# ai-forever/Kandinsky-2

Measured on AMD Instinct MI355X. Metric: UNet denoise steps/sec @ 768x768 bs=1, 50 steps, higher is better.
Workload: dtype bf16; 1 GPU; Kandinsky-2.x text2img 768x768, decoder_steps=50, bs=1/GPU (CFG batch 2x4x96x96), 2.1-architecture UNet (1.23B) p_sampler step; parity pinned against the reference's modules; head=2.1, tile_configs_measured_in_this_process=0, images_per_gpu=1, parallelism=prompt-sharded x1, weights by one RCCL broadcast, world_size_observed=1, graph=True, chains=1, loop_graph=a 5-step loop replayed as ONE hipGraph (83 replay(s) = 415 timed steps)

## Files before the change

### include/k22.h

```cpp
#ifndef K22_H
#define K22_H
#include <stddef.h>
#include <stdint.h>
#ifdef __cplusplus
extern "C" {
#endif

#define K22_OK 0
#define K22_EINVAL (-1)
#define K22_EHIP (-2)
#define K22_ENOMEM (-3)

#define K22_BF16 0
#define K22_F32 1
#define K22_F16 2
#define K22_F16X3 3
#define K22_F16X2 4

int k22_version(void);
#define K22_BUILD_PACKED_FP32 1
#define K22_BUILD_DEBUG_VARIANTS 2
int k22_build_flags(void);
const char* k22_last_error(void);
int k22_set_option(const char* name, int value);
// ... 12 lines not shown
  int n_levels;
  int channel_mult[8];
  int n_attention_ds;
  int attention_ds[8];
  int num_head_channels;
  int ctx_dim;
  int ctx_len;
  int n_image_embs;
  int text_dim1;
  int text_dim2;
  int image_dim;
  int head_type;
  int hint_channels;
} K22UNetConfig;

typedef struct K22Weight {
  const char* name;
  const void* ptr;
} K22Weight;

typedef struct K22UNet K22UNet;

int k22_unet_create(const K22UNetConfig* cfg, const K22Weight* weights, int n_weights, K22UNet** out);
void k22_unet_destroy(K22UNet* u);


int k22_unet_plan(K22UNet* u, int B, int H, int W, size_t* workspace_bytes);
int k22_unet_bind(K22UNet* u, void* workspace, size_t workspace_bytes);

int k22_unet_set_condition(K22UNet* u, const float* full_emb, const float* pooled_emb, const float* image_emb,
                           void* stream);

int k22_unet_set_hint(K22UNet* u, const float* hint, void* stream);

int k22_unet_forward(K22UNet* u, const float* x, const float* timesteps, const float* inpaint_image,
                     const float* inpaint_mask, float* out, int use_graph, void* stream);

int k22_unet_sample_loop(K22UNet* u, float* x, float* x_tmp, const float* timesteps, const float* noise_seq, const float* init_img,
                         const float* mask, const float* inpaint_image, const float* inpaint_mask, const float* table,
                         const int* table_rows, int n_steps, float guidance, float clamp_lo, float clamp_hi, int pct_index,
                         double pct_gamma, void* scratch, int use_graph, void* stream);
enum { K22_LOOP_DDIM = 0, K22_LOOP_PLMS = 1 };
int k22_unet_ddim_loop(K22UNet* u, int kind, float* x, float* x_tmp, float* x0_out, const float* timesteps, const float* table,
                       const float* noise_seq, const float* inpaint_image, const float* inpaint_mask, float* eps_hist, int n_steps,
                       float guidance, int use_graph, void* stream);
int k22_unet_num_ops(const K22UNet* u);
int k22_unet_set_autotune(K22UNet* u, int on);
int k22_unet_tuning_report(const K22UNet* u, char* buf, size_t cap);

int k22_comm_broadcast_weights(void* arena, size_t bytes, int root, void* nccl_comm, void* stream);

int k22_tile_table_load(const char* path);
int k22_tile_table_save(const char* path);
int k22_tile_table_size(void);
int k22_tile_table_measured(void);
void k22_tile_table_clear(void);

int k22_unet_profile(K22UNet* u, int reps, double* ms, double* flops, double* bytes, int* launches, void* stream);

size_t k22_sampler_scratch_bytes(int N, int HW);
int k22_ddim_step(const float* x, const float* model_out, const float* noise, const float* table_row, float guidance, int use_cfg,
                  float* x_out, float* x0_out, int N, int HW, void* stream);
int k22_prepare_mask(const float* mask, float* out, int C, int H, int W, void* stream);
int k22_plms_step(const float* x, const float* model_out, const float* eps_hist1, const float* eps_hist2, const float* eps_hist3, int order,
                  const float* table_row, float guidance, int use_cfg, float* x_out, float* eps_out, float* x0_out, int N, int HW, void* stream);
int k22_sampler_step(const float* x, const float* model_out, const float* noise, const float* init_img,
                     const float* mask, const float* table, int step_index, float guidance, int use_cfg,
                     float clamp_lo, float clamp_hi, int pct_index, double pct_gamma, void* scratch,
                     float* x_out, float* x0_out, int N, int HW, void* stream);

int k22_gemm(const void* A0, const void* A1, const void* Wp, const float* bias, const void* residual, void* out,
             void* partial, int M, int N, int Npad, int K0, int K1, long lda0, long lda1, int ldo, int ldr,
             int out_f32, int act, int splitk, int bm, int bn, int dtype, void* stream);
int k22_x3_pack(const float* src, void* dst, long n, float scale, void* stream);
int k22_conv3x3(const void* x_padded, const void* Wp, const float* bias, const void* residual, void* out,
                void* partial, int B, int H, int W, int Cin, int Cout, int Npad, int out_mode, int act, int splitk,
                int bm, int bn, int dtype, void* stream);
int k22_conv3x3_skip(const void* x_padded, const void* Wp, const float* bias, const void* skip0, const void* skip1,
                     int SK0, int SK1, const void* Ws, const float* bias_s, void* out, void* partial, int B, int H, int W,
                     int Cin, int Cout, int Npad, int splitk, int bm, int dtype, void* stream);
int k22_conv3x3_gnstats(const void* x_padded, const void* Wp, const float* bias, const void* residual, void* out,
                        void* partial, int B, int H, int W, int Cin, int Cout, int Npad, int splitk, int bm, int bn,
                        float* stats, int stats_capacity_rows, int* rows_per_image, int dtype, void* stream);
int k22_gemm_gnstats(const void* A, const void* Wp, const float* bias, const void* residual, void* out, void* partial,
                     int B, int H, int W, int N, int Npad, int K, int splitk, int bm, float* stats,
                     int stats_capacity_rows, int* rows_per_image, int dtype, void* stream);
typedef struct K22IgemmProblem {
  int dtype, taps, M, N, Kc, K0, H, W;
  int out_mode, res_f32, act, a_raw, want_stats;
  int SK0, SK1;
  int att_T, att_S, att_Tkp;
  int ldo, ldr;
  int has_frag;
  int algo, bm, bn, splitk, stages;
} K22IgemmProblem;
typedef struct K22IgemmOperands {
  const void *A0, *A1, *Wp, *bias, *residual;
  void *out, *partial;
  const void *S0, *S1, *Ws, *bias2;
  void *kall, *vtall;
  const void *Wfrag, *Wsfrag;
  float* stats;
  int stats_capacity_rows;
} K22IgemmOperands;
int k22_igemm_cfg_accepted(const K22IgemmProblem* pr);
int k22_igemm_cfg(const K22IgemmProblem* pr, const K22IgemmOperands* ops, int* rows_per_image, void* stream);
int k22_debug_conv_trace(const void* x_padded, const void* Wp, const float* bias, void* out, int B, int H, int W, int Cin, int Cout,
                         int Npad, unsigned long long* trace, void* stream);
int k22_conv3x3_gn(const void* x0, const void* x1, int C0, int C1, const float* gamma, const float* beta, const float* film, long film_ld,
                   float eps, int act, void* scratch, const void* Wp, const float* bias, const void* residual, void* out, void* partial,
                   int B, int H, int W, int Cout, int Npad, int splitk, int bm, int algo, int dtype, void* stream);
int k22_groupnorm(const void* x0, const void* x1, int C0, int C1, int B, int H, int W, const float* gamma,
                  const float* beta, const float* film, long film_ld, float eps, int act, int mode, int pad,
                  void* scratch, void* out, int dtype, void* stream);
size_t k22_groupnorm_scratch_bytes(int B, int C);
int k22_attention(const void* qkv, const void* ctxkv, void* kall, void* vtall, void* out, int B, int H, int T, int S,
                  int dtype, void* stream);
int k22_qkv_project(const void* x, const void* Wp, const float* bias, void* q_out, void* kall, void* vtall,
                    int B, int H, int T, int S, int K, int bm, int bn, int dtype, void* stream);
int k22_qkv_project_stream(const void* x, const void* Wp, const float* bias, void* q_out, void* kall, void* vtall, void* partial,
                           int B, int H, int T, int S, int K, int bm, int splitk, int dtype, void* stream);
int k22_linear_smallm(const float* x, const void* W, const float* bias, const float* add, float* out, int M, int N,
                      int K, int act_in, int act_out, int wdtype, void* stream);
int k22_conv3x3_direct(const float* x, const float* w, const float* bias, float* y, int B, int Cin, int Cout, int Hin, int Win,
                       int stride, int act, void* stream);

size_t k22_afrag_bytes(int M, int K);
int k22_afrag_pack(const void* A, long lda, void* out, int M, int K, int dtype, void* stream);
int k22_skinny_gemm(const void* Afrag, const void* Wfrag, const float* bias, void* out, float* partial, int M, int N, int Npad, int K,
                    int splitk, int epi, int act, int ldo, int mt, int nb, int dtype, void* stream);
int k22_finish_ln(const float* partial, int splitk, const float* bias, float* x, long ldx, const float* gain, const float* beta, void* yfrag,
                  int M, int N, float eps, int dtype, void* stream);
int k22_small_attention(const void* qkv, const float* qkv_partial, int nsplit, const float* qkv_bias, void* out, int out_frag, int B, int H, int T,
                        int causal, const float* key_valid, int kv_n, int dtype, void* stream);

typedef struct K22PriorConfig {
  int dtype;
  int text_ctx;
  int xf_width;
  int xf_layers;
  int xf_heads;
  int xf_final_ln;
  int clip_dim;
  int clip_xf_width;
} K22PriorConfig;
typedef struct K22Prior K22Prior;
int k22_prior_create(const K22PriorConfig* cfg, const K22Weight* weights, int n_weights, K22Prior** out);
void k22_prior_destroy(K22Prior* m);
int k22_prior_plan(K22Prior* m, int B, size_t* workspace_bytes);
int k22_prior_bind(K22Prior* m, void* workspace, size_t workspace_bytes);
int k22_prior_tuning_report(const K22Prior* m, char* buf, size_t cap);
int k22_prior_forward(K22Prior* m, const float* x, const float* timesteps, const float* text_emb, const float* text_enc,
                      const float* key_valid, float* out, void* stream);
int k22_prior_sampler_step(const float* x, const float* model_out, const float* noise, const float* scales, const float* table_row,
                           float clamp, float* x_out, int bs, int D, void* stream);

typedef struct K22MoVQConfig {
  int dtype;
  int ch;
  int n_levels;
  int ch_mult[8];
  int num_res_blocks;
  int attn_levels;
  int z_channels;
  int out_ch;
} K22MoVQConfig;
// ... 70 lines not shown
```

### kandinsky-2_amd/_lib.py

```python
from __future__ import annotations

import ctypes as C
import os

_HERE = os.path.dirname(os.path.abspath(__file__))
LIB_PATH = os.environ.get("K22_LIB_PATH") or os.path.join(_HERE, "libk22hip.so")
TILE_TABLE_PATH = os.path.join(_HERE, "tiles_gfx950.txt")

K22_BF16, K22_F32, K22_F16, K22_F16X3, K22_F16X2 = 0, 1, 2, 3, 4
K22_LOOP_DDIM, K22_LOOP_PLMS = 0, 1
F16X3 = "f16x3"
F16X2 = "f16x2"
SPLIT_DTYPES = (F16X3, F16X2)
X3_WSCALE = 256.0


def dtype_code(backend_dtype) -> int:
    import torch
    try:
        return {torch.bfloat16: K22_BF16, torch.float32: K22_F32, torch.float16: K22_F16, F16X3: K22_F16X3, F16X2: K22_F16X2}[backend_dtype]
    except KeyError:
        raise ValueError('backend_dtype must be torch.bfloat16, torch.float16, torch.float32 "f16x3" or "f16x2"') from None
ACT_NONE, ACT_SILU, ACT_GELU = 0, 1, 2
OUT_ROWMAJOR, OUT_ROWMAJOR_F32, OUT_NCHW_F32, OUT_QKV = 0, 1, 2, 3
# ... 23 lines not shown

class K22MoVQConfig(C.Structure):
    _fields_ = [("dtype", C.c_int), ("ch", C.c_int), ("n_levels", C.c_int), ("ch_mult", C.c_int * 8),
                ("num_res_blocks", C.c_int), ("attn_levels", C.c_int), ("z_channels", C.c_int), ("out_ch", C.c_int)]


class K22PriorConfig(C.Structure):
    _fields_ = [("dtype", C.c_int), ("text_ctx", C.c_int), ("xf_width", C.c_int), ("xf_layers", C.c_int), ("xf_heads", C.c_int),
                ("xf_final_ln", C.c_int), ("clip_dim", C.c_int), ("clip_xf_width", C.c_int)]


class K22EncoderConfig(C.Structure):
    _fields_ = [("dtype", C.c_int), ("kind", C.c_int), ("width", C.c_int), ("layers", C.c_int), ("heads", C.c_int), ("n_ctx", C.c_int),
                ("vocab", C.c_int), ("out_dim", C.c_int), ("image_size", C.c_int), ("patch", C.c_int), ("max_pos", C.c_int),
                ("pad_id", C.c_int), ("ln_eps", C.c_float), ("mlp_dim", C.c_int), ("hidden_act", C.c_int)]


class K22Weight(C.Structure):
    _fields_ = [("name", C.c_char_p), ("ptr", C.c_void_p)]


_P, _I, _L, _F, _D, _Z = C.c_void_p, C.c_int, C.c_long, C.c_float, C.c_double, C.c_size_t

SIGNATURES = {
    "k22_version": (_I, []),
    "k22_build_flags": (_I, []),
    "k22_last_error": (C.c_char_p, []),
    "k22_set_option": (_I, [C.c_char_p, _I]),
    "k22_comm_broadcast_weights": (_I, [_P, _Z, _I, _P, _P]),
    "k22_tile_table_load": (_I, [C.c_char_p]),
    "k22_tile_table_save": (_I, [C.c_char_p]),
    "k22_tile_table_size": (_I, []),
    "k22_tile_table_measured": (_I, []),
    "k22_tile_table_clear": (None, []),
    "k22_unet_create": (_I, [C.POINTER(K22UNetConfig), C.POINTER(K22Weight), _I, C.POINTER(_P)]),
    "k22_unet_destroy": (None, [_P]),
    "k22_unet_plan": (_I, [_P, _I, _I, _I, C.POINTER(_Z)]),
    "k22_unet_bind": (_I, [_P, _P, _Z]),
    "k22_unet_set_condition": (_I, [_P, _P, _P, _P, _P]),
    "k22_unet_set_hint": (_I, [_P, _P, _P]),
    "k22_unet_forward": (_I, [_P, _P, _P, _P, _P, _P, _I, _P]),
    "k22_unet_sample_loop": (_I, [_P, _P, _P, _P, _P, _P, _P, _P, _P, _P, C.POINTER(_I), _I, _F, _F, _F, _I, _D, _P, _I, _P]),
    "k22_unet_ddim_loop": (_I, [_P, _I, _P, _P, _P, _P, _P, _P, _P, _P, _P, _I, _F, _I, _P]),
    "k22_unet_num_ops": (_I, [_P]),
    "k22_unet_set_autotune": (_I, [_P, _I]),
    "k22_unet_tuning_report": (_I, [_P, C.c_char_p, _Z]),
    "k22_unet_profile": (_I, [_P, _I, C.POINTER(_D), C.POINTER(_D), C.POINTER(_D), C.POINTER(_I), _P]),
    "k22_afrag_bytes": (_Z, [_I, _I]),
    "k22_afrag_pack": (_I, [_P, _L, _P, _I, _I, _I, _P]),
    "k22_skinny_gemm": (_I, [_P, _P, _P, _P, _P, _I, _I, _I, _I, _I, _I, _I, _I, _I, _I, _I, _P]),
    "k22_finish_ln": (_I, [_P, _I, _P, _P, _L, _P, _P, _P, _I, _I, _F, _I, _P]),
    "k22_small_attention": (_I, [_P, _P, _I, _P, _P, _I, _I, _I, _I, _I, _P, _I, _I, _P]),
    "k22_prior_create": (_I, [C.POINTER(K22PriorConfig), C.POINTER(K22Weight), _I, C.POINTER(_P)]),
    "k22_prior_destroy": (None, [_P]),
    "k22_prior_plan": (_I, [_P, _I, C.POINTER(_Z)]),
    "k22_prior_bind": (_I, [_P, _P, _Z]),
    "k22_prior_tuning_report": (_I, [_P, C.c_char_p, _Z]),
    "k22_prior_forward": (_I, [_P, _P, _P, _P, _P, _P, _P, _P]),
    "k22_prior_sampler_step": (_I, [_P, _P, _P, _P, _P, _F, _P, _I, _I, _P]),
    "k22_encoder_create": (_I, [C.POINTER(K22EncoderConfig), C.POINTER(K22Weight), _I, C.POINTER(_P)]),
    "k22_encoder_destroy": (None, [_P]),
    "k22_encoder_plan": (_I, [_P, _I, C.POINTER(_Z)]),
    "k22_encoder_bind": (_I, [_P, _P, _Z]),
    "k22_encoder_forward": (_I, [_P, _P, _P, _P, _P, _P, _P]),
    "k22_movq_create": (_I, [C.POINTER(K22MoVQConfig), C.POINTER(K22Weight), _I, C.POINTER(_P)]),
    "k22_movq_destroy": (None, [_P]),
    "k22_movq_plan": (_I, [_P, _I, _I, _I, C.POINTER(_Z)]),
    "k22_movq_bind": (_I, [_P, _P, _Z]),
    "k22_movq_decode": (_I, [_P, _P, _P, _P, _P]),
    "k22_movq_plan_encoder": (_I, [_P, _I, _I, _I, C.POINTER(_Z)]),
    "k22_movq_encode": (_I, [_P, _P, _P, _P]),
    "k22_movq_num_ops": (_I, [_P]),
    "k22_ddim_step": (_I, [_P, _P, _P, _P, _F, _I, _P, _P, _I, _I, _P]),
    "k22_blend_noised": (_I, [_P, _P, _P, _P, _F, _F, _P, _I, _I, _I, _I, _P]),
    "k22_prepare_mask": (_I, [_P, _P, _I, _I, _I, _P]),
    "k22_plms_step": (_I, [_P, _P, _P, _P, _P, _I, _P, _F, _I, _P, _P, _P, _I, _I, _P]),
    "k22_sampler_scratch_bytes": (_Z, [_I, _I]),
    "k22_sampler_step": (_I, [_P, _P, _P, _P, _P, _P, _I, _F, _I, _F, _F, _I, _D, _P, _P, _P, _I, _I, _P]),
    "k22_gemm": (_I, [_P, _P, _P, _P, _P, _P, _P, _I, _I, _I, _I, _I, _L, _L, _I, _I, _I, _I, _I, _I, _I, _I, _P]),
    "k22_x3_pack": (_I, [_P, _P, _L, _F, _P]),
    "k22_conv3x3": (_I, [_P, _P, _P, _P, _P, _P, _I, _I, _I, _I, _I, _I, _I, _I, _I, _I, _I, _I, _P]),
    "k22_conv3x3_skip": (_I, [_P, _P, _P, _P, _P, _I, _I, _P, _P, _P, _P, _I, _I, _I, _I, _I, _I, _I, _I, _I, _P]),
    "k22_gemm_gnstats": (_I, [_P, _P, _P, _P, _P, _P, _I, _I, _I, _I, _I, _I, _I, _I, _P, _I, C.POINTER(_I), _I, _P]),
    "k22_conv3x3_gnstats": (_I, [_P, _P, _P, _P, _P, _P, _I, _I, _I, _I, _I, _I, _I, _I, _I, _P, _I, C.POINTER(_I), _I, _P]),
    "k22_igemm_cfg_accepted": (_I, [C.POINTER(K22IgemmProblem)]),
    "k22_igemm_cfg": (_I, [C.POINTER(K22IgemmProblem), C.POINTER(K22IgemmOperands), C.POINTER(_I), _P]),
    "k22_conv3x3_gn": (_I, [_P, _P, _I, _I, _P, _P, _P, _L, _F, _I, _P, _P, _P, _P, _P, _P, _I, _I, _I, _I, _I, _I, _I, _I, _I, _P]),
    "k22_debug_conv_trace": (_I, [_P, _P, _P, _P, _I, _I, _I, _I, _I, _I, _P, _P]),
    "k22_groupnorm": (_I, [_P, _P, _I, _I, _I, _I, _I, _P, _P, _P, _L, _F, _I, _I, _I, _P, _P, _I, _P]),
    "k22_groupnorm_scratch_bytes": (_Z, [_I, _I]),
    "k22_attention": (_I, [_P, _P, _P, _P, _P, _I, _I, _I, _I, _I, _P]),
    "k22_qkv_project": (_I, [_P, _P, _P, _P, _P, _P, _I, _I, _I, _I, _I, _I, _I, _I, _P]),
    "k22_qkv_project_stream": (_I, [_P, _P, _P, _P, _P, _P, _P, _I, _I, _I, _I, _I, _I, _I, _I, _P]),
    "k22_linear_smallm": (_I, [_P, _P, _P, _P, _P, _I, _I, _I, _I, _I, _I, _P]),
    "k22_conv3x3_direct": (_I, [_P, _P, _P, _P, _I, _I, _I, _I, _I, _I, _I, _P]),
    "k22_debug_counter": (_L, [C.c_char_p]),
    "k22_stream_frag_bytes": (C.c_size_t, [_I, _I, _I, _I]),
    "k22_stream_repack": (_I, [_P, _P, _I, _I, _I, _I, _P]),
    "k22_debug_set_stream_frag": (_I, [_P, _P]),
    "k22_debug_set_stream_scratch": (_I, [_P, C.c_size_t]),
    "k22_spatialnorm_apply": (_I, [_P, _P, _P, _P, _P, _P, _P, _P, _I, _I, _I, _I, _I, _I, _I, _I, _I, _I, _P]),
    "k22_upsample2_pad": (_I, [_P, _P, _I, _I, _I, _I, _I, _P]),
    "k22_pad_copy": (_I, [_P, _P, _I, _I, _I, _I, _I, _P]),
    "k22_subsample_odd": (_I, [_P, _P, _I, _I, _I, _I, _I, _P]),
    "k22_softmax_rows": (_I, [_P, _L, _I, _F, _I, _P]),
    "k22_movq_prepare": (_I, [_P, _P, _P, _P, _P, _I, _I, _I, _I, _I, _P]),
    "k22_movq_enc_prepare": (_I, [_P, _P, _I, _I, _I, _I, _I, _P]),
    "k22_movq_quant_conv": (_I, [_P, _P, _P, _P, _I, _I, _P]),
    "k22_to_uint8_nhwc": (_I, [_P, _P, _I, _I, _I, _I, _P]),
    "k22_enc_layernorm": (_I, [_P, _L, _P, _P, _P, _L, _P, _I, _I, _F, _I, _P]),
    "k22_enc_embed": (_I, [_P, _P, _P, _P, _P, _I, _I, _I, _I, _I, _I, _I, _P]),
    "k22_enc_gather_eot": (_I, [_P, _P, _P, _I, _I, _I, _P]),
    "k22_enc_masked_mean": (_I, [_P, _P, _P, _I, _I, _I, _P]),
    "k22_enc_patchify": (_I, [_P, _P, _I, _I, _I, _I, _I, _P]),
    "k22_enc_vision_assemble": (_I, [_P, _P, _P, _P, _I, _I, _I, _P]),
    "k22_enc_mlp_act": (_I, [_P, _P, _L, _I, _I, _P]),
    "k22_enc_attention_generic": (_I, [_P, _P, _I, _I, _I, _I, _I, _P]),
    "k22_prior_layernorm": (_I, [_P, _L, _P, _P, _P, _I, _I, _I, _I, _P]),
    "k22_prior_finish_input": (_I, [_P, _P, _P, _I, _I, _I, _P]),
    "k22_attention_masked": (_I, [_P, _P, _P, _P, _P, _I, _I, _I, _I, _I, _P, _I, _I, _I, _P]),
}

_lib = None


def lib() -> C.CDLL:
    global _lib
    if _lib is None:
        if not os.path.exists(LIB_PATH):
            raise RuntimeError(
                f"{LIB_PATH} is missing: the HIP extension is the only compute path (no CPU fallback). "
                "Build it with `python -c 'import __graft_entry__ as g; g.build()'`.")
        l = C.CDLL(LIB_PATH)
        for name, (res, args) in SIGNATURES.items():
            fn = getattr(l, name)
            fn.restype = res
            fn.argtypes = args
        _lib = l
        tbl = os.environ.get("K22_TILE_TABLE", TILE_TABLE_PATH)
        if tbl != "0" and os.path.exists(tbl):
            if l.k22_tile_table_load(tbl.encode()) < 0:
                raise RuntimeError(f"k22: cannot read the tile table {tbl}")
    return _lib


def check(rc: int) -> None:
    if rc != 0:
        msg = lib().k22_last_error()
        raise RuntimeError(f"k22 error {rc}: {msg.decode() if msg else ''}")


def weight_array(arena, table):
    base = arena.data_ptr()
    arr = (K22Weight * len(table))()
    names = []
    for i, (name, (off, _n)) in enumerate(table.items()):
        nb = name.encode()
        names.append(nb)
        arr[i].name = nb
        arr[i].ptr = base + off
    return arr, names


def plan_and_bind(plan_fn, bind_fn, handle, device, *shape):
    import torch
    nbytes = C.c_size_t()
# ... 17 lines not shown
```

### kandinsky-2_amd/csrc/capi.hip

```cpp
#include "kernels.h"
#include "elementwise.h"
#include "../../include/k22.h"
#include "tuning.h"
#include "skinny.h"
#include <dlfcn.h>
#include <stdio.h>
#include <string.h>

static thread_local char g_err[512] = "";

int k22_set_error(int code, const char* msg) {
  snprintf(g_err, sizeof(g_err), "%s", msg ? msg : "");
  return code;
}
int k22_set_error_hip(hipError_t e, const char* file, int line) {
  snprintf(g_err, sizeof(g_err), "HIP error %d (%s) at %s:%d", (int)e, hipGetErrorString(e), file, line);
  return K22_EHIP;
}

extern "C" {

int k22_version(void) { return 100; }
int k22_build_flags(void) {
  int f = 0;
#ifndef K22_NOPK
  f |= K22_BUILD_PACKED_FP32;
#endif
#if defined(K22_DEBUG_VARIANTS) || defined(K22_STREAM_DEBUG) || defined(K22_SKINNY_DEBUG)
  f |= K22_BUILD_DEBUG_VARIANTS;
#endif
  return f;
}

int k22_set_option(const char* name, int value) {
  if (name && !strcmp(name, "igemm_stages")) { igemm_set_default_stages(value); return K22_OK; }
  if (name && !strcmp(name, "igemm_xcd_remap")) { igemm_set_xcd_remap(value); return K22_OK; }
  if (name && !strcmp(name, "conv_algo")) { igemm_set_conv_algo(value); return K22_OK; }
  if (name && !strcmp(name, "gemm_algo")) { igemm_set_gemm_algo(value); return K22_OK; }
  if (name && !strcmp(name, "att_pipe")) { attention_set_pipe(value); return K22_OK; }
  return k22_set_error(K22_EINVAL, "k22_set_option: unknown option");
}
const char* k22_last_error(void) { return g_err; }

#ifdef K22_STREAM_DEBUG
static unsigned long long* g_dbg_trace = nullptr;
extern "C" int k22_debug_set_stream_trace(unsigned long long* t) { g_dbg_trace = t; return K22_OK; }
#define K22_DBG_TRACE(p) (p).st_trace = g_dbg_trace
#else
#define K22_DBG_TRACE(p) (void)0
#endif
static const void* g_dbg_wfrag = nullptr;
static const void* g_dbg_wsfrag = nullptr;
static void* g_dbg_scratch = nullptr;
static size_t g_dbg_scratch_bytes = 0;
static int dbg_frag(IgemmParams& p, int dtype, hipStream_t st) {
  K22_DBG_TRACE(p);
  p.Wfrag = g_dbg_wfrag; p.Wsfrag = g_dbg_wsfrag;
  if (g_dbg_wfrag || !g_dbg_scratch || dtype == K22_F32 || (p.taps != 1 && p.taps != 9) || p.Kc % 64 || p.Npad % 64) return K22_OK;
  const size_t n1 = stream_frag_bytes(p.Npad, p.taps, p.Kc, dtype);
  const bool skip = p.S0 != nullptr && p.Ws != nullptr && (p.SK0 + p.SK1) % 64 == 0;
  const size_t n2 = skip ? stream_frag_bytes(p.Npad, 1, p.SK0 + p.SK1, dtype) : 0;
  if (n1 + n2 > g_dbg_scratch_bytes) return k22_set_error(K22_ENOMEM, "debug stream scratch too small");
  if (int rc = launch_stream_repack(p.Wp, g_dbg_scratch, p.Npad, p.taps, p.Kc, dtype, st)) return rc;
  p.Wfrag = g_dbg_scratch;
  if (skip) {
    void* w2 = static_cast<char*>(g_dbg_scratch) + n1;
    if (int rc = launch_stream_repack(p.Ws, w2, p.Npad, 1, p.SK0 + p.SK1, dtype, st)) return rc;
    p.Wsfrag = w2;
  }
  return K22_OK;
}
#define K22_DBG_FRAG(p) do { if (int rc_ = dbg_frag((p), dtype, reinterpret_cast<hipStream_t>(stream))) return rc_; } while (0)
int k22_debug_set_stream_frag(const void* wfrag, const void* wsfrag) { g_dbg_wfrag = wfrag; g_dbg_wsfrag = wsfrag; return K22_OK; }
int k22_debug_set_stream_scratch(void* scratch, size_t bytes) { g_dbg_scratch = scratch; g_dbg_scratch_bytes = scratch ? bytes : 0; return K22_OK; }
size_t k22_stream_frag_bytes(int Npad, int taps, int Kc, int dtype) { return stream_frag_bytes(Npad, taps, Kc, dtype); }
int k22_stream_repack(const void* W, void* out, int Npad, int taps, int Kc, int dtype, void* stream) {
  return launch_stream_repack(W, out, Npad, taps, Kc, dtype, reinterpret_cast<hipStream_t>(stream));
}

long k22_debug_counter(const char* name) {
  if (name && !strcmp(name, "stream_launches")) return stream_launch_count();
  if (name && !strcmp(name, "loop_captures")) return loop_capture_count();
  if (name && !strcmp(name, "loop_launches")) return loop_launch_count();
  return -1;
}

int k22_comm_broadcast_weights(void* arena, size_t bytes, int root, void* nccl_comm, void* stream) {
  if (!arena || !nccl_comm) return k22_set_error(K22_EINVAL, "k22_comm_broadcast_weights: null arena / communicator");
  typedef int (*bcast_fn)(const void*, void*, size_t, int , int, void*, hipStream_t);
  static bcast_fn fn = nullptr;
  if (!fn) {
    void* sym = dlsym(RTLD_DEFAULT, "ncclBroadcast");
    if (!sym) {
      void* h = dlopen("librccl.so.1", RTLD_NOW | RTLD_GLOBAL);
      if (!h) h = dlopen("librccl.so", RTLD_NOW | RTLD_GLOBAL);
      if (h) sym = dlsym(h, "ncclBroadcast");
    }
    if (!sym) return k22_set_error(K22_EINVAL, "k22_comm_broadcast_weights: RCCL (ncclBroadcast) is not loadable in this process");
    fn = reinterpret_cast<bcast_fn>(sym);
  }
  const size_t piece = (size_t)1 << 30;
  char* base = reinterpret_cast<char*>(arena);
  for (size_t off = 0; off < bytes; off += piece) {
    const size_t n = bytes - off < piece ? bytes - off : piece;
    const int rc = fn(base + off, base + off, n,  1, root, nccl_comm, reinterpret_cast<hipStream_t>(stream));
    if (rc != 0) { char msg[96]; snprintf(msg, sizeof msg, "k22_comm_broadcast_weights: ncclBroadcast returned %d", rc); return k22_set_error(K22_EHIP, msg); }
  }
  return K22_OK;
}

int k22_tile_table_load(const char* path) {
  if (!path) return k22_set_error(K22_EINVAL, "k22_tile_table_load: null path");
  const int n = tile_table_load_file(path);
  if (n < 0) return k22_set_error(K22_EINVAL, "k22_tile_table_load: cannot read the file");
  return n;
}
int k22_tile_table_save(const char* path) {
  if (!path) return k22_set_error(K22_EINVAL, "k22_tile_table_save: null path");
  const int n = tile_table_save_file(path);
  if (n < 0) return k22_set_error(K22_EINVAL, "k22_tile_table_save: cannot write the file");
  return n;
}
int k22_tile_table_size(void) {
  TileTable& tt = tile_table();
  std::lock_guard<std::mutex> lk(tt.mu);
  return (int)tt.m.size();
}
int k22_tile_table_measured(void) {
  TileTable& tt = tile_table();
  std::lock_guard<std::mutex> lk(tt.mu);
  return (int)tt.measured;
}
void k22_tile_table_clear(void) {
  TileTable& tt = tile_table();
  std::lock_guard<std::mutex> lk(tt.mu);
  tt.m.clear();
  tt.measured = 0;
}

int k22_gemm(const void* A0, const void* A1, const void* Wp, const float* bias, const void* residual, void* out,
             void* partial, int M, int N, int Npad, int K0, int K1, long lda0, long lda1, int ldo, int ldr,
             int out_f32, int act, int splitk, int bm, int bn, int dtype, void* stream) {
  IgemmParams p = igemm_gemm_problem(M, N, K0, K1, out_f32 ? IG_OUT_ROWMAJOR_F32 : IG_OUT_ROWMAJOR, act);
  p.A0 = A0; p.A1 = A1; p.Wp = Wp; p.bias = bias; p.residual = residual; p.out = out;
  p.partial = reinterpret_cast<float*>(partial);
  p.Npad = Npad; p.lda0 = lda0; p.lda1 = lda1; p.ldo = ldo; p.ldr = ldr;
  p.splitk = splitk; p.force_bm = bm; p.force_bn = bn;
  p.a_raw = k22_is_split(dtype) ? 1 : 0;
  if (p.splitk == 0) p.splitk = partial ? igemm_choose_splitk(p, dtype) : 1;
  K22_DBG_FRAG(p);
  return launch_igemm(p, dtype, reinterpret_cast<hipStream_t>(stream));
}

int k22_x3_pack(const float* src, void* dst, long n, float scale, void* stream) {
  if (!src || !dst || n < 0) return k22_set_error(K22_EINVAL, "x3_pack: null argument");
  return launch_x3_pack(src, dst, n, scale, reinterpret_cast<hipStream_t>(stream));
}

int k22_conv3x3(const void* x_padded, const void* Wp, const float* bias, const void* residual, void* out,
                void* partial, int B, int H, int W, int Cin, int Cout, int Npad, int out_mode, int act, int splitk,
                int bm, int bn, int dtype, void* stream) {
  IgemmParams p = igemm_conv3_problem(B, H, W, Cin, Cout, out_mode, act);
  p.A0 = x_padded; p.Wp = Wp; p.bias = bias; p.residual = residual; p.out = out;
  p.partial = reinterpret_cast<float*>(partial);
  p.Npad = Npad; p.splitk = splitk; p.force_bm = bm; p.force_bn = bn;
  if (p.splitk == 0) p.splitk = partial ? igemm_choose_splitk(p, dtype) : 1;
  K22_DBG_FRAG(p);
  return launch_igemm(p, dtype, reinterpret_cast<hipStream_t>(stream));
}

int k22_conv3x3_gnstats(const void* x_padded, const void* Wp, const float* bias, const void* residual, void* out,
                        void* partial, int B, int H, int W, int Cin, int Cout, int Npad, int splitk, int bm, int bn,
                        float* stats, int stats_capacity_rows, int* rows_per_image, int dtype, void* stream) {
  IgemmParams p = igemm_conv3_problem(B, H, W, Cin, Cout);
  p.A0 = x_padded; p.Wp = Wp; p.bias = bias; p.residual = residual; p.out = out;
  p.partial = reinterpret_cast<float*>(partial);
  p.Npad = Npad; p.splitk = splitk; p.force_bm = bm; p.force_bn = bn;
  if (p.splitk == 0) p.splitk = partial ? igemm_choose_splitk(p, dtype) : 1;
  const int rpi = igemm_stats_rows_per_image(p, dtype);
  if (rows_per_image) *rows_per_image = rpi;
  if (rpi <= 0) return k22_set_error(K22_EINVAL, "conv3x3_gnstats: this configuration cannot produce GroupNorm partial sums");
  if (rpi * B > stats_capacity_rows) return k22_set_error(K22_ENOMEM, "conv3x3_gnstats: stats buffer too small");
  p.stats = stats;
  K22_DBG_FRAG(p);
  return launch_igemm(p, dtype, reinterpret_cast<hipStream_t>(stream));
}

int k22_gemm_gnstats(const void* A, const void* Wp, const float* bias, const void* residual, void* out, void* partial,
                     int B, int H, int W, int N, int Npad, int K, int splitk, int bm, float* stats,
                     int stats_capacity_rows, int* rows_per_image, int dtype, void* stream) {
  IgemmParams p = igemm_gemm_problem(B * H * W, N, K, 0);
  p.A0 = A; p.Wp = Wp; p.bias = bias; p.residual = residual; p.out = out; p.partial = reinterpret_cast<float*>(partial);
  p.Npad = Npad; p.H = H; p.W = W;
  p.splitk = splitk > 0 ? splitk : 1;
  p.force_bm = bm; p.algo = (bm == 160 || bm == 288) ? IG_ALGO_STREAM : IG_ALGO_GEMM8;
  p.a_raw = k22_is_split(dtype) ? 1 : 0;
  const int rpi = igemm_stats_rows_per_image(p, dtype);
  if (rows_per_image) *rows_per_image = rpi;
  if (rpi <= 0) return k22_set_error(K22_EINVAL, "gemm_gnstats: this configuration cannot produce GroupNorm partial sums");
  if (rpi * B > stats_capacity_rows) return k22_set_error(K22_ENOMEM, "gemm_gnstats: stats buffer too small");
  p.stats = stats;
  K22_DBG_FRAG(p);
  return launch_igemm(p, dtype, reinterpret_cast<hipStream_t>(stream));
}

int k22_conv3x3_skip(const void* x_padded, const void* Wp, const float* bias, const void* skip0, const void* skip1,
                     int SK0, int SK1, const void* Ws, const float* bias_s, void* out, void* partial, int B, int H, int W,
                     int Cin, int Cout, int Npad, int splitk, int bm, int dtype, void* stream) {
  IgemmParams p = igemm_conv3_problem(B, H, W, Cin, Cout);
  p.A0 = x_padded; p.Wp = Wp; p.bias = bias; p.out = out; p.partial = reinterpret_cast<float*>(partial);
  p.Npad = Npad; p.splitk = splitk; p.force_bm = bm;
  p.S0 = skip0; p.S1 = skip1; p.SK0 = SK0; p.SK1 = SK1; p.Ws = Ws; p.bias2 = bias_s;
  if (p.splitk == 0) p.splitk = partial ? igemm_choose_splitk(p, dtype) : 1;
  K22_DBG_FRAG(p);
  return launch_igemm(p, dtype, reinterpret_cast<hipStream_t>(stream));
}

static int igemm_problem_tuned(const K22IgemmProblem& d, Tuned& t) {
  if (d.dtype < K22_BF16 || d.dtype > K22_F16X2) return k22_set_error(K22_EINVAL, "igemm_cfg: bad dtype");
  if ((d.taps != 1 && d.taps != 9) || d.M <= 0 || d.N <= 0 || d.Kc <= 0 || d.K0 <= 0 || d.K0 > d.Kc)
    return k22_set_error(K22_EINVAL, "igemm_cfg: bad problem (taps 1 / 9, M, N > 0, 0 < K0 <= Kc)");
  if (d.out_mode < IG_OUT_ROWMAJOR || d.out_mode > IG_OUT_QKV || d.SK0 < 0 || d.SK1 < 0 || (d.SK1 > 0 && d.SK0 == 0))
    return k22_set_error(K22_EINVAL, "igemm_cfg: bad output mode / skip widths");
  if (d.taps == 9 && (d.H <= 0 || d.W <= 0 || d.M % (d.H * d.W))) return k22_set_error(K22_EINVAL, "igemm_cfg: a convolution needs M = B * H * W");
  const void* mark = reinterpret_cast<const void*>(1);
  IgemmParams& p = t.p;
  if (d.taps == 9) {
    p = igemm_conv3_problem(d.M / (d.H * d.W), d.H, d.W, d.Kc, d.N, d.out_mode, d.act);
    p.K0 = d.K0;
  } else {
    p = igemm_gemm_problem(d.M, d.N, d.K0, d.Kc - d.K0, d.out_mode, d.act);
    p.H = d.H; p.W = d.W;
  }
  p.ldo = d.ldo > 0 ? d.ldo : (d.out_mode == IG_OUT_QKV ? d.N / 3 : d.N);
  p.ldr = d.ldr > 0 ? d.ldr : (d.res_f32 ? p.ldo : d.N);
  p.res_f32 = d.res_f32 ? 1 : 0; p.a_raw = d.a_raw ? 1 : 0;
  p.Wp = mark; p.bias = reinterpret_cast<const float*>(mark);
  if (d.SK0 > 0) { p.S0 = mark; p.S1 = d.SK1 > 0 ? mark : nullptr; p.SK0 = d.SK0; p.SK1 = d.SK1; p.Ws = mark; p.bias2 = reinterpret_cast<const float*>(mark); }
  if (d.out_mode == IG_OUT_QKV) { p.att_T = d.att_T; p.att_S = d.att_S; p.att_Tkp = d.att_Tkp; }
  if (d.has_frag) { p.Wfrag = mark; if (d.SK0 > 0) p.Wsfrag = mark; }
  t.want_stats = d.want_stats != 0;
  t.dt = d.dtype;
  tuned_make_candidates(t, d.dtype);
  return K22_OK;
}
static Cfg igemm_problem_cfg(const K22IgemmProblem& d) {
  Cfg c; c.algo = d.algo; c.bm = d.bm; c.bn = d.bn; c.splitk = d.splitk; c.stages = d.stages;
  return c;
}

int k22_igemm_cfg_accepted(const K22IgemmProblem* pr) {
  if (!pr) return k22_set_error(K22_EINVAL, "igemm_cfg_accepted: null problem");
  Tuned t;
  if (int rc = igemm_problem_tuned(*pr, t)) return rc;
  return tuned_is_candidate(t, igemm_problem_cfg(*pr)) ? 1 : 0;
}

int k22_igemm_cfg(const K22IgemmProblem* pr, const K22IgemmOperands* ops, int* rows_per_image, void* stream) {
  if (rows_per_image) *rows_per_image = 0;
  if (!pr || !ops) return k22_set_error(K22_EINVAL, "igemm_cfg: null problem / operands");
  const K22IgemmProblem& d = *pr;
  const K22IgemmOperands& o = *ops;
  Tuned t;
  if (int rc = igemm_problem_tuned(d, t)) return rc;
  const Cfg c = igemm_problem_cfg(d);
  if (!tuned_is_candidate(t, c)) return k22_set_error(K22_EINVAL, "igemm_cfg: this build does not generate the configuration for the problem");
  if (!o.A0 || !o.Wp || !o.out) return k22_set_error(K22_EINVAL, "igemm_cfg: A0, Wp and out are required");
  if (d.K0 < d.Kc && !o.A1) return k22_set_error(K22_EINVAL, "igemm_cfg: A1 missing for the concat operand");
// ... 274 lines not shown
```

### kandinsky-2_amd/csrc/elementwise.h

```cpp
#pragma once
#include "common.h"

struct GnStatsParams {
  const void* x0; const void* x1;
  int C0, C1, HW, B, groups, nsplit;
  float* partial;
};
struct GnSrc { const float* st; int rpi, C; };
struct GnCoeffParams {
  GnSrc src[2];
  int HW, C, groups; float eps;
  const float* gamma; const float* beta;
  const float* film; int64_t film_ld;
  float* coeff;
};
struct GnApplyParams {
  const void* x0; const void* x1; int C0, C1;
  int B, H, W;
  int mode;
  int pad;
  int act;
  const float* coeff;
  void* out;
  int out_x3;
};
struct ConvInParams {
  const float* x; const float* img; const float* mask;
  const float* w; const float* bias;
  void* out;
  int B, H, W, Cin, Cout;
  int img_premul;
};
struct ConvDirectParams {
  const float* x; const float* w; const float* bias; float* y;
  int B, Cin, Cout, Hin, Win, stride, act;
};
int launch_conv3x3_direct(const ConvDirectParams& p, hipStream_t s);
struct LinearSmallParams {
  const float* x; int64_t ldx;
  const void* W;
  const float* bias;
  const float* add; int64_t ld_add;
  int add_mod;
  float* out; int64_t ldo;
  int M, N, K, act_in, act_out;
  int rows_per_wave;
};
struct KvPackParams {
  const void* qkv; const void* ctxkv; void* kall; void* vtall;
  int B, H, T, S, Tkp;
};
struct AttentionParams {
  const void* q; int64_t ldq;
  const void* kall; const void* vtall;
  void* out; int64_t ldo;
  int B, H, T, Tk, Tkp;
  float scale;
  int causal;
  const float* key_valid;
  int kv_ld, kv_n;
  int out_x3;
};
struct SmallAttnParams {
  const void* qkv; int64_t ldq;
  const float* part; int nsplit; const float* bias;
  void* out; int64_t ldo;
  int out_frag, MA;
  int B, H, T;
  float scale;
  int causal;
  const float* key_valid; int kv_ld, kv_n;
};
struct SamplerParams {
  const float* x;
  const float* model_out;
  const float* noise;
  const float* init_img;
  const float* mask;
  const float* table;
  const int* step;
  int step_host;
  float guidance, clamp_lo, clamp_hi;
  int use_cfg;
  int n_lo; double gamma;
  float* x0_buf;
  float* s_buf;
  float* x_out;
  float* x0_out;
  int N, HW;
};

int launch_x3_pack(const float* in, void* out, int64_t n, float scale, hipStream_t s);
int gn_nsplit(int B, int HW);
int launch_gn_stats(const GnStatsParams& p, int dtype, hipStream_t s);
int launch_gn_coeff(const GnCoeffParams& p, int B, hipStream_t s);
inline int launch_gn_stats_coeff(const void* x0, const void* x1, int C0, int C1, int B, int HW, float eps, const float* gamma, const float* beta,
                                 const float* film, int64_t film_ld, float* partial, float* coeff, int dtype, hipStream_t s) {
  const int nsplit = gn_nsplit(B, HW), C = C0 + C1;
  GnStatsParams sp = {};
  sp.x0 = x0; sp.x1 = x1; sp.C0 = C0; sp.C1 = C1; sp.HW = HW; sp.B = B; sp.groups = 32; sp.nsplit = nsplit; sp.partial = partial;
  const int rc = launch_gn_stats(sp, dtype, s);
  if (rc) return rc;
  GnCoeffParams cp = {};
  cp.src[0].st = partial; cp.src[0].rpi = nsplit; cp.src[0].C = C;
  cp.HW = HW; cp.C = C; cp.groups = 32; cp.eps = eps; cp.gamma = gamma; cp.beta = beta; cp.film = film; cp.film_ld = film_ld; cp.coeff = coeff;
  return launch_gn_coeff(cp, B, s);
}
int launch_gn_apply(const GnApplyParams& p, int dtype, hipStream_t s);
int launch_resample(const void* x, void* y, int B, int H, int W, int C, int mode, int dtype, hipStream_t s);
int launch_conv_in(const ConvInParams& p, int dtype, hipStream_t s);
int launch_timestep_embedding(const float* t, const float* freqs, float* out, int B, int half, hipStream_t s);
int launch_linear_smallm(const LinearSmallParams& p, int wdtype, hipStream_t s);
int launch_layernorm_f32(const float* x, const float* g, const float* b, float* y, int rows, int D, float eps, hipStream_t s);
int launch_cast_rows(const float* x, void* y, int rows, int cols, int64_t ldx, int64_t ldy, int dtype, hipStream_t s);
int launch_kv_pack(const KvPackParams& p, int dtype, hipStream_t s);
int launch_attention(const AttentionParams& p, int dtype, hipStream_t s);
int launch_small_attention(const SmallAttnParams& p, int dtype, hipStream_t s);
int launch_sampler_step(const SamplerParams& p, hipStream_t s);
int launch_plms_step(const float* x, const float* model_out, const float* h1, const float* h2, const float* h3, int order, const float* tab,
                     float guidance, int use_cfg, float* x_out, float* e_store, float* x0_out, int N, int HW, hipStream_t s);
int launch_prepare_mask(const float* old_mask, float* out, int C, int H, int W, hipStream_t s);
int launch_ddim_step(const float* x, const float* model_out, const float* noise, const float* tab, float guidance, int use_cfg,
                     float* x_out, float* x0_out, int N, int HW, hipStream_t s);

struct SpatialNormParams {
  const void* x;
  const float* coeff;
  const float* zq;
  const float* wy; const float* by;
  const float* wb; const float* bb;
  void* out;
  int B, H, W, C, h0, w0, shift, act, pad;
};
int launch_spatialnorm_apply(const SpatialNormParams& p, int dtype, hipStream_t s);
int launch_upsample2_pad(const void* x, void* y, int B, int H, int W, int C, int dtype, hipStream_t s);
int launch_softmax_rows(void* x, int64_t rows, int L, float scale, int dtype, hipStream_t s);
int launch_movq_prepare(const float* z, const float* wpq, const float* bpq, float* zq, void* xin, int B, int h, int w,
                        int Cpad, int dtype, hipStream_t s);
int launch_movq_enc_prepare(const float* img, void* xin, int B, int H, int W, int Cpad, int dtype, hipStream_t s);
int launch_pad_copy(const void* x, void* y, int B, int H, int W, int C, int dtype, hipStream_t s);
int launch_subsample_odd(const void* x, void* y, int B, int H, int W, int C, int dtype, hipStream_t s);
int launch_movq_quant_conv(const float* h, const float* wq, const float* bq, float* out, int B, int HW, hipStream_t s);
int launch_to_uint8_nhwc(const float* x, unsigned char* y, int B, int C, int H, int W, hipStream_t s);
```

### kandinsky-2_amd/csrc/elementwise.hip

```cpp
#include "kernels.h"
#include "elementwise.h"

__device__ __forceinline__ void load4(const bf16_t* p, float* f) {
  const uint2 r = *reinterpret_cast<const uint2*>(p);
  f[0] = __uint_as_float(r.x << 16); f[1] = __uint_as_float(r.x & 0xffff0000u);
  f[2] = __uint_as_float(r.y << 16); f[3] = __uint_as_float(r.y & 0xffff0000u);
}
__device__ __forceinline__ void load4(const f16_t* p, float* f) {
  const uint2 r = *reinterpret_cast<const uint2*>(p);
  unpack2_f16(r.x, f[0], f[1]); unpack2_f16(r.y, f[2], f[3]);
}
__device__ __forceinline__ void load4(const float* p, float* f) {
  const float4 r = *reinterpret_cast<const float4*>(p);
  f[0] = r.x; f[1] = r.y; f[2] = r.z; f[3] = r.w;
}

template <typename T>
__global__ __launch_bounds__(256) void gn_stats_kernel(GnStatsParams p) {
  __shared__ float red[1024 * 2 * 2];
  const int tid = threadIdx.x, b = blockIdx.y, s = blockIdx.x;
  const int C = p.C0 + p.C1, VP = C / 4;
  const int per = (p.HW + p.nsplit - 1) / p.nsplit;
  const int pix0 = s * per, pix1 = min(p.HW, pix0 + per);
  const T* x0 = reinterpret_cast<const T*>(p.x0) + (int64_t)b * p.HW * p.C0;
  const T* x1 = p.x1 ? reinterpret_cast<const T*>(p.x1) + (int64_t)b * p.HW * p.C1 : nullptr;
  int PL, pl;
  if (VP >= 256) { PL = 1; pl = 0; } else { PL = 256 / VP; pl = tid / VP; }
  float sum[3][4], sq[3][4];
  int vj[3];
#pragma unroll
  for (int j = 0; j < 3; ++j) {
    int v = (VP >= 256) ? tid + 256 * j : ((j == 0 && pl < PL) ? tid - pl * VP : VP);
    vj[j] = v < VP ? v : -1;
#pragma unroll
    for (int k = 0; k < 4; ++k) { sum[j][k] = 0.f; sq[j][k] = 0.f; }
  }
#pragma unroll
  for (int j = 0; j < 3; ++j) {
    if (vj[j] >= 0) {
      const int c = vj[j] * 4;
      const T* src = c < p.C0 ? x0 + c : x1 + (c - p.C0);
      const int64_t ld = c < p.C0 ? p.C0 : p.C1;
      int pix = pix0 + pl;
      for (; pix + 7 * PL < pix1; pix += 8 * PL) {
        float f[8][4];
#pragma unroll
        for (int u = 0; u < 8; ++u) load4(src + (int64_t)(pix + u * PL) * ld, f[u]);
#pragma unroll
        for (int k = 0; k < 4; ++k) {
          sum[j][k] += ((f[0][k] + f[1][k]) + (f[2][k] + f[3][k])) + ((f[4][k] + f[5][k]) + (f[6][k] + f[7][k]));
          sq[j][k] += ((f[0][k] * f[0][k] + f[1][k] * f[1][k]) + (f[2][k] * f[2][k] + f[3][k] * f[3][k])) +
                      ((f[4][k] * f[4][k] + f[5][k] * f[5][k]) + (f[6][k] * f[6][k] + f[7][k] * f[7][k]));
        }
      }
      for (; pix < pix1; pix += PL) {
        float f[4];
        load4(src + (int64_t)pix * ld, f);
#pragma unroll
        for (int k = 0; k < 4; ++k) { sum[j][k] += f[k]; sq[j][k] += f[k] * f[k]; }
      }
    }
  }
  float* out = p.partial + ((int64_t)b * p.nsplit + s) * C * 2;
  if (PL == 1) {
#pragma unroll
    for (int j = 0; j < 3; ++j)
      if (vj[j] >= 0) {
        float* o = out + (int64_t)vj[j] * 8;
        *reinterpret_cast<float4*>(o) = make_float4(sum[j][0], sq[j][0], sum[j][1], sq[j][1]);
        *reinterpret_cast<float4*>(o + 4) = make_float4(sum[j][2], sq[j][2], sum[j][3], sq[j][3]);
      }
    return;
  }
  if (vj[0] >= 0) {
    float* o = red + ((int64_t)pl * C + vj[0] * 4) * 2;
    *reinterpret_cast<float4*>(o) = make_float4(sum[0][0], sq[0][0], sum[0][1], sq[0][1]);
    *reinterpret_cast<float4*>(o + 4) = make_float4(sum[0][2], sq[0][2], sum[0][3], sq[0][3]);
  }
  __syncthreads();
  for (int i = tid; i < C * 2; i += 256) {
    float a = 0.f;
    for (int q = 0; q < PL; ++q) a += red[(int64_t)q * C * 2 + i];
    out[i] = a;
  }
// ... 93 lines not shown
  if (xo < 0 || yo < 0 || xo >= Wo || yo >= Ho) {
#pragma unroll
    for (int k = 0; k < EPV / 2; ++k) o.set2(k, 0.f, 0.f);
  } else {
    const int c = cv * EPV;
    const T* src; int cs, ld;
    if (c < p.C0) { src = reinterpret_cast<const T*>(p.x0); cs = c; ld = p.C0; }
    else { src = reinterpret_cast<const T*>(p.x1); cs = c - p.C0; ld = p.C1; }
    float A[EPV], Bc[EPV];
    const float* cf = p.coeff + ((int64_t)b * C + c) * 2;
#pragma unroll
    for (int k = 0; k < EPV; k += 2) {
      const float4 q = *reinterpret_cast<const float4*>(cf + 2 * k);
      A[k] = q.x; Bc[k] = q.y; A[k + 1] = q.z; Bc[k + 1] = q.w;
    }
    float r[EPV];
    if (p.mode == 1) {
      Vec16<T> v[4];
#pragma unroll
      for (int dy = 0; dy < 2; ++dy)
#pragma unroll
        for (int dx = 0; dx < 2; ++dx)
          v[dy * 2 + dx].raw = *reinterpret_cast<const decltype(v[0].raw)*>(src + ((int64_t)(b * p.H + 2 * yo + dy) * p.W + 2 * xo + dx) * ld + cs);
#pragma unroll
      for (int k = 0; k < EPV; ++k) {
        float acc = 0.f;
#pragma unroll
        for (int q = 0; q < 4; ++q) acc += fast ? apply_act_sel<true>(v[q].get(k) * A[k] + Bc[k], p.act) : apply_act_sel<false>(v[q].get(k) * A[k] + Bc[k], p.act);
        r[k] = acc * 0.25f;
      }
    } else {
      const int yi = p.mode == 2 ? yo >> 1 : yo, xi = p.mode == 2 ? xo >> 1 : xo;
      Vec16<T> v;
      v.raw = *reinterpret_cast<const decltype(v.raw)*>(src + ((int64_t)(b * p.H + yi) * p.W + xi) * ld + cs);
#pragma unroll
      for (int k = 0; k < EPV; ++k) r[k] = fast ? apply_act_sel<true>(v.get(k) * A[k] + Bc[k], p.act) : apply_act_sel<false>(v.get(k) * A[k] + Bc[k], p.act);
    }
#pragma unroll
    for (int k = 0; k < EPV / 2; ++k) o.set2(k, r[2 * k], r[2 * k + 1]);
  }
  if constexpr (sizeof(T) == 4) {
    if (p.out_x3) { x3_store4(out, x3_split4(o.raw)); return; }
  }
  *reinterpret_cast<decltype(o.raw)*>(out) = o.raw;
}

template <typename T>
__global__ __launch_bounds__(256) void resample_kernel(const void* xin, void* yout, int B, int H, int W, int C, int mode) {
  constexpr int EPV = Vec16<T>::N;
  const int CV = C / EPV;
  const int Ho = mode == 1 ? H / 2 : H * 2, Wo = mode == 1 ? W / 2 : W * 2;
  const int64_t total = (int64_t)B * Ho * Wo * CV;
  const T* x = reinterpret_cast<const T*>(xin);
  T* y = reinterpret_cast<T*>(yout);
  for (int64_t i = (int64_t)blockIdx.x * 256 + threadIdx.x; i < total; i += (int64_t)gridDim.x * 256) {
    const int cv = (int)(i % CV);
    int64_t t = i / CV;
    const int xo = (int)(t % Wo); t /= Wo;
    const int yo = (int)(t % Ho);
    const int b = (int)(t / Ho);
    Vec16<T> o;
    if (mode == 1) {
      float r[EPV];
#pragma unroll
      for (int k = 0; k < EPV; ++k) r[k] = 0.f;
#pragma unroll
      for (int dy = 0; dy < 2; ++dy)
#pragma unroll
        for (int dx = 0; dx < 2; ++dx) {
          Vec16<T> v;
          v.raw = *reinterpret_cast<const decltype(v.raw)*>(x + ((int64_t)(b * H + 2 * yo + dy) * W + 2 * xo + dx) * C + cv * EPV);
#pragma unroll
          for (int k = 0; k < EPV; ++k) r[k] += v.get(k);
        }
#pragma unroll
      for (int k = 0; k < EPV / 2; ++k) o.set2(k, r[2 * k] * 0.25f, r[2 * k + 1] * 0.25f);
    } else {
      o.raw = *reinterpret_cast<const decltype(o.raw)*>(x + ((int64_t)(b * H + (yo >> 1)) * W + (xo >> 1)) * C + cv * EPV);
    }
    *reinterpret_cast<decltype(o.raw)*>(y + i * EPV) = o.raw;
  }
}

constexpr int CONV_IN_PT = 8;
template <typename T, int CIN>
__global__ __launch_bounds__(128) void conv_in_kernel(ConvInParams p) {
  constexpr int PT = CONV_IN_PT, PW = PT + 2;
  __shared__ float patch[CIN][3][PW];
  const int tid = threadIdx.x;
  const int xt = blockIdx.x, y = blockIdx.y, b = blockIdx.z;
  const int x0 = xt * PT;
  const int hw = p.H * p.W;
  for (int i = tid; i < CIN * 3 * PW; i += 128) {
    const int c = i / (3 * PW), r = (i / PW) % 3, xx = i % PW;
    const int yy = y + r - 1, xs = x0 + xx - 1;
    float v = 0.f;
    if (yy >= 0 && yy < p.H && xs >= 0 && xs < p.W) {
      const int64_t o = (int64_t)yy * p.W + xs;
      if (c < 4) v = p.x[((int64_t)b * 4 + c) * hw + o];
      else if (c < 8) v = p.img[((int64_t)b * 4 + (c - 4)) * hw + o] * (p.img_premul ? 1.f : p.mask[(int64_t)b * hw + o]);
      else v = p.mask[(int64_t)b * hw + o];
    }
    patch[c][r][xx] = v;
  }
  __syncthreads();
  T* out = reinterpret_cast<T*>(p.out);
  for (int n = tid; n < p.Cout; n += 128) {
    float w[CIN * 9];
#pragma unroll
    for (int k = 0; k < CIN * 9; ++k) w[k] = p.w[(int64_t)k * p.Cout + n];
    const float bias = p.bias[n];
    for (int px = 0; px < PT && x0 + px < p.W; ++px) {
      float acc = bias;
#pragma unroll
      for (int c = 0; c < CIN; ++c)
#pragma unroll
        for (int r = 0; r < 3; ++r)
#pragma unroll
          for (int q = 0; q < 3; ++q) acc += w[c * 9 + r * 3 + q] * patch[c][r][px + q];
      out[((int64_t)(b * p.H + y) * p.W + x0 + px) * p.Cout + n] = from_f32<T>(acc);
    }
  }
}

template <int OCB>
__global__ __launch_bounds__(256) void conv3x3_direct_kernel(ConvDirectParams p) {
  const int Ho = (p.Hin - 1) / p.stride + 1, Wo = (p.Win - 1) / p.stride + 1;
  const int pix = blockIdx.x * 256 + threadIdx.x;
  const int oc0 = blockIdx.y * OCB, b = blockIdx.z;
  if (pix >= Ho * Wo) return;
  const int yo = pix / Wo, xo = pix - yo * Wo;
  const int yi = yo * p.stride - 1, xi = xo * p.stride - 1;
  float acc[OCB];
#pragma unroll
  for (int o = 0; o < OCB; ++o) acc[o] = (oc0 + o < p.Cout) ? p.bias[oc0 + o] : 0.f;
  const int64_t plane = (int64_t)p.Hin * p.Win;
  for (int c = 0; c < p.Cin; ++c) {
    const float* xp = p.x + ((int64_t)b * p.Cin + c) * plane;
    float v[9];
#pragma unroll
    for (int r = 0; r < 3; ++r)
#pragma unroll
      for (int q = 0; q < 3; ++q) {
        const int yy = yi + r, xx = xi + q;
        v[r * 3 + q] = (yy >= 0 && yy < p.Hin && xx >= 0 && xx < p.Win) ? xp[(int64_t)yy * p.Win + xx] : 0.f;
      }
#pragma unroll
    for (int o = 0; o < OCB; ++o) {
      if (oc0 + o < p.Cout) {
        const float* wp = p.w + ((int64_t)(oc0 + o) * p.Cin + c) * 9;
#pragma unroll
        for (int k = 0; k < 9; ++k) acc[o] += wp[k] * v[k];
      }
    }
  }
#pragma unroll
  for (int o = 0; o < OCB; ++o)
    if (oc0 + o < p.Cout) p.y[(((int64_t)b * p.Cout + oc0 + o) * Ho + yo) * Wo + xo] = apply_act(acc[o], p.act);
}

__global__ void timestep_embedding_kernel(const float* t, const float* freqs, float* out, int B, int half) {
  const int i = blockIdx.x * blockDim.x + threadIdx.x;
  if (i >= B * half) return;
  const int b = i / half, k = i - b * half;
  const float a = t[b] * freqs[k];
  out[(int64_t)b * 2 * half + k] = cosf(a);
  out[(int64_t)b * 2 * half + half + k] = sinf(a);
}

// ... 55 lines not shown
  if ((tid & 63) == 0) red[tid >> 6] = s;
  __syncthreads();
  const float mean = (red[0] + red[1] + red[2] + red[3]) / D;
  float q = 0.f;
  for (int i = tid; i < D; i += 256) { const float d = xr[i] - mean; q += d * d; }
  q = wave_sum(q);
  if ((tid & 63) == 0) red[4 + (tid >> 6)] = q;
  __syncthreads();
  const float rstd = rsqrtf((red[4] + red[5] + red[6] + red[7]) / D + eps);
  for (int i = tid; i < D; i += 256) y[(int64_t)row * D + i] = (xr[i] - mean) * rstd * g[i] + bta[i];
}

template <typename T>
__global__ void cast_rows_kernel(const float* x, void* yout, int rows, int cols, int64_t ldx, int64_t ldy) {
  T* y = reinterpret_cast<T*>(yout);
  const int64_t total = (int64_t)rows * cols;
  for (int64_t i = (int64_t)blockIdx.x * blockDim.x + threadIdx.x; i < total; i += (int64_t)gridDim.x * blockDim.x) {
    const int r = (int)(i / cols), c = (int)(i - (int64_t)r * cols);
    y[r * ldy + c] = from_f32<T>(x[r * ldx + c]);
  }
}

template <typename T>
__global__ __launch_bounds__(256) void kv_pack_kernel(KvPackParams p) {
  __shared__ T vt[64][66];
  const int tid = threadIdx.x, jt = blockIdx.x, h = blockIdx.y, b = blockIdx.z;
  const int C = p.H * 64, Tk = p.S + p.T;
  const T* qkv = reinterpret_cast<const T*>(p.qkv);
  const T* ckv = reinterpret_cast<const T*>(p.ctxkv);
  T* Kall = reinterpret_cast<T*>(p.kall) + ((int64_t)(b * p.H + h) * p.Tkp) * 64;
  T* VTall = reinterpret_cast<T*>(p.vtall) + ((int64_t)(b * p.H + h) * 64) * p.Tkp;
  for (int i = tid; i < 64 * 64; i += 256) {
    const int jj = i >> 6, d = i & 63;
    const int j = jt * 64 + jj;
    T kv = from_f32<T>(0.f), vv = from_f32<T>(0.f);
    if (j < p.S) {
      const T* r = ckv + (int64_t)(b * p.S + j) * 2 * C + h * 64 + d;
      kv = r[0]; vv = r[C];
    } else if (j < Tk) {
      const T* r = qkv + (int64_t)(b * p.T + (j - p.S)) * 3 * C + C + h * 64 + d;
      kv = r[0]; vv = r[C];
    }
    Kall[(int64_t)j * 64 + d] = kv;
    vt[d][jj] = vv;
  }
  __syncthreads();
  for (int i = tid; i < 64 * 64; i += 256) {
    const int d = i >> 6, jj = i & 63;
    VTall[(int64_t)d * p.Tkp + jt * 64 + jj] = vt[d][jj];
  }
}

__global__ __launch_bounds__(256) void x3_pack_kernel(const float4* __restrict__ in, u32x4_t* __restrict__ out, int64_t n4, float scale) {
  for (int64_t i = (int64_t)blockIdx.x * 256 + threadIdx.x; i < n4; i += (int64_t)gridDim.x * 256) {
    const float4 v = in[i];
    x3_store4(out + i, x3_split4(v.x * scale, v.y * scale, v.z * scale, v.w * scale));
  }
}
int launch_x3_pack(const float* in, void* out, int64_t n, float scale, hipStream_t s) {
  if (n % 8 || (uintptr_t)in % 16 || (uintptr_t)out % 32) return k22_set_error(K22_EINVAL, "x3_pack: n % 8 == 0, 16-byte aligned input, 32-byte aligned output (groups of eight)");
  const int64_t n4 = n / 4;
  int nb = (int)((n4 + 255) / 256);
  if (nb > 4096) nb = 4096;
  if (nb < 1) return K22_OK;
  hipLaunchKernelGGL(x3_pack_kernel, dim3(nb), dim3(256), 0, s, reinterpret_cast<const float4*>(in), reinterpret_cast<u32x4_t*>(out), n4, scale);
  K22_CHECK_LAUNCH();
  return K22_OK;
}

static inline int grid_for(int64_t total, int threads, int cap) {
  int64_t nb = (total + threads - 1) / threads;
  if (nb > cap) nb = cap;
  if (nb < 1) nb = 1;
  return (int)nb;
}

int gn_nsplit(int B, int HW) {
  int ns = 512 / (B > 0 ? B : 1);
  if (ns > 128) ns = 128;
  while (ns > 1 && HW / ns < 32) ns >>= 1;
  return ns < 1 ? 1 : ns;
}

int launch_gn_stats(const GnStatsParams& p, int dtype, hipStream_t s) {
  const int C = p.C0 + p.C1;
  if (p.groups != 32 || C % 128 != 0 || p.C0 % 4 != 0) return k22_set_error(K22_EINVAL, "gn_stats: need 32 groups, C % 128 == 0");
  if (C / 4 > 768) return k22_set_error(K22_EINVAL, "gn_stats: C too large (max 3072)");
  if (C / 4 < 256 && (256 / (C / 4)) * C > 2048) return k22_set_error(K22_EINVAL, "gn_stats: internal LDS bound");
  dim3 grid(p.nsplit, p.B);
  if (dtype == K22_BF16) hipLaunchKernelGGL(gn_stats_kernel<bf16_t>, grid, dim3(256), 0, s, p);
  else if (dtype == K22_F16) hipLaunchKernelGGL(gn_stats_kernel<f16_t>, grid, dim3(256), 0, s, p);
  else hipLaunchKernelGGL(gn_stats_kernel<float>, grid, dim3(256), 0, s, p);
  K22_CHECK_LAUNCH();
  return K22_OK;
}
int launch_gn_coeff(const GnCoeffParams& p, int B, hipStream_t s) {
  if (p.C / p.groups > 256) return k22_set_error(K22_EINVAL, "gn_coeff: more than 256 channels per group");
  hipLaunchKernelGGL(gn_coeff_kernel, dim3(p.groups, B), dim3(256), 0, s, p);
  K22_CHECK_LAUNCH();
  return K22_OK;
}
int launch_gn_apply(const GnApplyParams& p, int dtype, hipStream_t s) {
  const int C = p.C0 + p.C1;
  const int epv = dtype == K22_F32 ? 4 : 8;
  if (C % epv || p.C0 % epv) return k22_set_error(K22_EINVAL, "gn_apply: channel alignment");
  if (p.out_x3 && dtype != K22_F32) return k22_set_error(K22_EINVAL, "gn_apply: x3-chunk output is an option of the fp32 launch");
  const int Ho = p.mode == 1 ? p.H / 2 : (p.mode == 2 ? p.H * 2 : p.H);
  const int Wo = p.mode == 1 ? p.W / 2 : (p.mode == 2 ? p.W * 2 : p.W);
  const int Hp = Ho + 2 * p.pad, Wp = Wo + 2 * p.pad;
  if (Hp > 65535 || p.B > 65535) return k22_set_error(K22_EINVAL, "gn_apply: tensor too large");
  dim3 grid((Wp * (C / epv) + 255) / 256, Hp, p.B);
  if (dtype == K22_BF16) hipLaunchKernelGGL(gn_apply_kernel<bf16_t>, grid, dim3(256), 0, s, p);
  else if (dtype == K22_F16) hipLaunchKernelGGL(gn_apply_kernel<f16_t>, grid, dim3(256), 0, s, p);
  else hipLaunchKernelGGL(gn_apply_kernel<float>, grid, dim3(256), 0, s, p);
  K22_CHECK_LAUNCH();
  return K22_OK;
}
int launch_resample(const void* x, void* y, int B, int H, int W, int C, int mode, int dtype, hipStream_t s) {
  const int epv = dtype == K22_F32 ? 4 : 8;
  const int Ho = mode == 1 ? H / 2 : H * 2, Wo = mode == 1 ? W / 2 : W * 2;
  const int nb = grid_for((int64_t)B * Ho * Wo * (C / epv), 256, 8192);
  if (dtype == K22_BF16) hipLaunchKernelGGL(resample_kernel<bf16_t>, dim3(nb), dim3(256), 0, s, x, y, B, H, W, C, mode);
  else if (dtype == K22_F16) hipLaunchKernelGGL(resample_kernel<f16_t>, dim3(nb), dim3(256), 0, s, x, y, B, H, W, C, mode);
  else hipLaunchKernelGGL(resample_kernel<float>, dim3(nb), dim3(256), 0, s, x, y, B, H, W, C, mode);
  K22_CHECK_LAUNCH();
  return K22_OK;
}
int launch_conv_in(const ConvInParams& p, int dtype, hipStream_t s) {
  dim3 grid((p.W + CONV_IN_PT - 1) / CONV_IN_PT, p.H, p.B);
  if (p.Cin == 4) {
    if (dtype == K22_BF16) hipLaunchKernelGGL((conv_in_kernel<bf16_t, 4>), grid, dim3(128), 0, s, p);
    else if (dtype == K22_F16) hipLaunchKernelGGL((conv_in_kernel<f16_t, 4>), grid, dim3(128), 0, s, p);
    else hipLaunchKernelGGL((conv_in_kernel<float, 4>), grid, dim3(128), 0, s, p);
  } else if (p.Cin == 9) {
    if (dtype == K22_BF16) hipLaunchKernelGGL((conv_in_kernel<bf16_t, 9>), grid, dim3(128), 0, s, p);
    else if (dtype == K22_F16) hipLaunchKernelGGL((conv_in_kernel<f16_t, 9>), grid, dim3(128), 0, s, p);
    else hipLaunchKernelGGL((conv_in_kernel<float, 9>), grid, dim3(128), 0, s, p);
  } else if (p.Cin == 8) {
    if (dtype == K22_BF16) hipLaunchKernelGGL((conv_in_kernel<bf16_t, 8>), grid, dim3(128), 0, s, p);
    else if (dtype == K22_F16) hipLaunchKernelGGL((conv_in_kernel<f16_t, 8>), grid, dim3(128), 0, s, p);
    else hipLaunchKernelGGL((conv_in_kernel<float, 8>), grid, dim3(128), 0, s, p);
  } else {
    return k22_set_error(K22_EINVAL, "conv_in: in_channels must be 4, 8 or 9");
  }
  K22_CHECK_LAUNCH();
  return K22_OK;
}
int launch_conv3x3_direct(const ConvDirectParams& p, hipStream_t s) {
  if (p.stride != 1 && p.stride != 2) return k22_set_error(K22_EINVAL, "conv3x3_direct: stride must be 1 or 2");
  const int Ho = (p.Hin - 1) / p.stride + 1, Wo = (p.Win - 1) / p.stride + 1;
  constexpr int OCB = 8;
  dim3 grid((Ho * Wo + 255) / 256, (p.Cout + OCB - 1) / OCB, p.B);
  hipLaunchKernelGGL((conv3x3_direct_kernel<OCB>), grid, dim3(256), 0, s, p);
  K22_CHECK_LAUNCH();
  return K22_OK;
}
int launch_timestep_embedding(const float* t, const float* freqs, float* out, int B, int half, hipStream_t s) {
  hipLaunchKernelGGL(timestep_embedding_kernel, dim3((B * half + 255) / 256), dim3(256), 0, s, t, freqs, out, B, half);
  K22_CHECK_LAUNCH();
  return K22_OK;
}
template <typename TW>
static void launch_linear_m(const LinearSmallParams& p, int Mt, dim3 grid, size_t smem, hipStream_t s) {
  switch (Mt) {
    case 1: hipLaunchKernelGGL((linear_smallm_kernel<TW, 1>), grid, dim3(256), smem, s, p); break;
    case 2: hipLaunchKernelGGL((linear_smallm_kernel<TW, 2>), grid, dim3(256), smem, s, p); break;
    case 4: hipLaunchKernelGGL((linear_smallm_kernel<TW, 4>), grid, dim3(256), smem, s, p); break;
    default: hipLaunchKernelGGL((linear_smallm_kernel<TW, 8>), grid, dim3(256), smem, s, p); break;
  }
}
int launch_linear_smallm(const LinearSmallParams& p0, int wdtype, hipStream_t s) {
  if (p0.M > 8 || p0.M < 1) return k22_set_error(K22_EINVAL, "linear_smallm: M must be in 1..8");
  const int epc = wdtype == K22_F32 ? 4 : 8;
  if (p0.K % epc) return k22_set_error(K22_EINVAL, "linear_smallm: K alignment");
  const int Mt = p0.M <= 2 ? p0.M : (p0.M <= 4 ? 4 : 8);
  const size_t smem = (size_t)Mt * p0.K * 4;
  if (smem > 64 * 1024) return k22_set_error(K22_EINVAL, "linear_smallm: M*K too large for the LDS stage");
  LinearSmallParams p = p0;
  int rpw = 1;
  while (rpw < 8 && (p.N + 8 * rpw - 1) / (8 * rpw) >= 1024) rpw *= 2;
  p.rows_per_wave = rpw;
  dim3 grid((p.N + 4 * rpw - 1) / (4 * rpw));
  if (wdtype == K22_BF16) launch_linear_m<bf16_t>(p, Mt, grid, smem, s);
  else if (wdtype == K22_F16) launch_linear_m<f16_t>(p, Mt, grid, smem, s);
  else launch_linear_m<float>(p, Mt, grid, smem, s);
  K22_CHECK_LAUNCH();
  return K22_OK;
}
int launch_layernorm_f32(const float* x, const float* g, const float* b, float* y, int rows, int D, float eps, hipStream_t s) {
  hipLaunchKernelGGL(layernorm_f32_kernel, dim3(rows), dim3(256), 0, s, x, g, b, y, D, eps);
  K22_CHECK_LAUNCH();
  return K22_OK;
}
int launch_cast_rows(const float* x, void* y, int rows, int cols, int64_t ldx, int64_t ldy, int dtype, hipStream_t s) {
  const int nb = grid_for((int64_t)rows * cols, 256, 4096);
  if (dtype == K22_BF16) hipLaunchKernelGGL(cast_rows_kernel<bf16_t>, dim3(nb), dim3(256), 0, s, x, y, rows, cols, ldx, ldy);
  else if (dtype == K22_F16) hipLaunchKernelGGL(cast_rows_kernel<f16_t>, dim3(nb), dim3(256), 0, s, x, y, rows, cols, ldx, ldy);
  else hipLaunchKernelGGL(cast_rows_kernel<float>, dim3(nb), dim3(256), 0, s, x, y, rows, cols, ldx, ldy);
  K22_CHECK_LAUNCH();
  return K22_OK;
}
int launch_kv_pack(const KvPackParams& p, int dtype, hipStream_t s) {
  if (p.Tkp % 64) return k22_set_error(K22_EINVAL, "kv_pack: Tkp % 64");
  dim3 grid(p.Tkp / 64, p.H, p.B);
  if (dtype == K22_BF16) hipLaunchKernelGGL(kv_pack_kernel<bf16_t>, grid, dim3(256), 0, s, p);
  else if (dtype == K22_F16) hipLaunchKernelGGL(kv_pack_kernel<f16_t>, grid, dim3(256), 0, s, p);
  else hipLaunchKernelGGL(kv_pack_kernel<float>, grid, dim3(256), 0, s, p);
  K22_CHECK_LAUNCH();
  return K22_OK;
}
```

### kandinsky-2_amd/csrc/engine.hip

```cpp
#include "kernels.h"
#include "elementwise.h"
#include "../../include/k22.h"
#include "tuning.h"
#include "plan.h"

#include <atomic>
#include <deque>
#include <functional>
#include <map>
#include <memory>
#include <string>
#include <tuple>
#include <unordered_map>
#include <vector>
#include <stdio.h>
#include <stdlib.h>
#include <string.h>

int launch_step_advance(int* step, int delta, hipStream_t s);

static std::atomic<long> g_loop_captures{0}, g_loop_launches{0};
long loop_capture_count() { return g_loop_captures.load(); }
long loop_launch_count() { return g_loop_launches.load(); }
static void loop_count_capture() { g_loop_captures.fetch_add(1); }
static void loop_count_launch() { g_loop_launches.fetch_add(1); }
enum : unsigned long long { K22_LOOP_KIND_P = 0, K22_LOOP_KIND_DDIM = 1, K22_LOOP_KIND_PLMS = 2 };
static unsigned long long loop_key_ptr(const void* p) { return (unsigned long long)(uintptr_t)p; }
static unsigned long long loop_key_bits(double v) { unsigned long long b; memcpy(&b, &v, 8); return b; }

namespace {

enum OpKind { OP_CONV3 = 0, OP_GEMM = 1, OP_GN = 2, OP_ATTN = 3, OP_MISC = 4, OP_NKINDS = 5 };

struct Op {
  std::function<int(hipStream_t)> fn;
  int kind = OP_MISC;
  double flops = 0.0;
  double flops2 = 0.0;
  double bytes = 0.0;
  int kernels = 1;
  Op() {}
  template <typename F> Op(F f, int k = OP_MISC, double fl = 0.0, double by = 0.0, int nk = 1) : fn(f), kind(k), flops(fl), bytes(by), kernels(nk) {}
  int operator()(hipStream_t st) const { return fn(st); }
};
typedef std::vector<Op> OpList;

struct Act {
  Slot* s0 = nullptr; int C0 = 0;
  Slot* s1 = nullptr; int C1 = 0;
  int H = 0, W = 0;
  const Tuned* p0 = nullptr; Slot* st0 = nullptr;
  const Tuned* p1 = nullptr; Slot* st1 = nullptr;
  int C() const { return C0 + C1; }
};

}

struct K22UNet : GraphPlan {
  K22UNetConfig cfg;
  int sdt;

  int B = 0, H = 0, W = 0;
  OpList ops;
  OpList cond_ops;
  OpList hint_ops;
  bool hint_set = false;
  int fuse_skip = 1;
  int fuse_gn = 0;
  struct GnLink { const Tuned* consumer = nullptr; };
  std::deque<GnLink> gn_links;
  int stream_frag = 1;
  struct FragJob { const void* W; Slot* slot; int Npad, taps, Kc; };
  std::vector<FragJob> frag_jobs;
  bool frag_done = false;
  int repack_frags(hipStream_t st) {
    for (auto& j : frag_jobs) {
      int rc = launch_stream_repack(j.W, ptr(j.slot), j.Npad, j.taps, j.Kc, dtype, st);
      if (rc) return rc;
    }
    frag_done = true;
    return K22_OK;
  }
  bool cond_set = false;
  GraphCache loop;
  std::vector<unsigned long long> loop_key;

  Slot *s_xin, *s_img, *s_mask, *s_t, *s_out;
  Slot *s_temb, *s_e1, *s_emb, *s_film, *s_xfproj, *s_ctx;
  Slot *s_full, *s_pool, *s_imgemb, *s_tmpf, *s_tmpf2, *s_fullT;
  Slot *s_part, *s_coeff, *s_P1, *s_U1, *s_P2, *s_S, *s_N, *s_QKV, *s_KALL, *s_VT, *s_ATT, *s_splitk, *s_flush;
  Slot *s_U1st;
  Slot *s_ctxf = nullptr, *s_hint = nullptr, *s_hintin = nullptr, *s_hbuf[2] = {nullptr, nullptr};
  Slot* s_h[3];
  Slot* s_hst[3];
  std::vector<Slot*> s_ctxkv;
  int n_attn = 0;
  int64_t film_total = 0;
  float* film_all = nullptr;
  size_t film_all_bytes = 0;
  int hoist_time = 1;
  const float* film_cur = nullptr;
  const float* film_base() const { return film_cur ? film_cur : ptr<float>(s_film); }
  struct TimeW { const float* freqs; const float* w0; const float* b0; const float* w2; const float* b2; const void* we; const float* be; int mc, ted, dt; } tw = {};
  int time_rows(const float* t, float* temb, float* e1, float* emb, float* film, int rows, hipStream_t st) {
    int rc = launch_timestep_embedding(t, tw.freqs, temb, rows, tw.mc / 2, st);
    if (rc) return rc;
    LinearSmallParams lp = {};
    lp.x = temb; lp.ldx = tw.mc; lp.W = tw.w0; lp.bias = tw.b0; lp.out = e1; lp.ldo = tw.ted;
    lp.M = rows; lp.N = tw.ted; lp.K = tw.mc; lp.act_in = K22_ACT_NONE; lp.act_out = K22_ACT_SILU;
    rc = launch_linear_smallm(lp, K22_F32, st);
    if (rc) return rc;
    lp.x = e1; lp.ldx = tw.ted; lp.W = tw.w2; lp.bias = tw.b2; lp.add = ptr<float>(s_xfproj); lp.ld_add = tw.ted; lp.add_mod = B;
    lp.out = emb; lp.K = tw.ted; lp.act_out = K22_ACT_NONE;
    rc = launch_linear_smallm(lp, K22_F32, st);
    if (rc) return rc;
    LinearSmallParams le = {};
    le.x = emb; le.ldx = tw.ted; le.W = tw.we; le.bias = tw.be; le.out = film; le.ldo = film_total;
    le.M = rows; le.N = (int)film_total; le.K = tw.ted; le.act_in = K22_ACT_SILU; le.act_out = K22_ACT_NONE;
    return launch_linear_smallm(le, tw.dt, st);
  }

  float* model_out() { return ptr<float>(s_out); }
  int exec(hipStream_t st) { return run_ops(st); }
  int exec_eager(hipStream_t st) { return run_eager(st, [this](hipStream_t s) { return exec(s); }); }
  int prepare_run(hipStream_t st) {
    if (!frag_done) { int rc = repack_frags(st); if (rc) return rc; }
    return tune_once(s_flush, st);
  }

  ~K22UNet() {
    if (film_all) (void)hipFree(film_all);
  }

  struct LoopRows {
    bool hoist = false;
    float *film = nullptr, *temb = nullptr, *e1 = nullptr, *emb = nullptr;
  };
  int loop_begin(int n_calls, hipStream_t st, LoopRows* lr) {
    if (int rc = prepare_run(st)) return rc;
    lr->hoist = B <= 8 && hoist_time;
    if (!lr->hoist) return K22_OK;
    const int64_t rows_all = (int64_t)n_calls * B;
    const size_t need = (size_t)rows_all * (size_t)(film_total + tw.mc + 2 * tw.ted) * sizeof(float);
    if (need > film_all_bytes) {
      loop.drop();
      if (film_all) { (void)hipStreamSynchronize(st); (void)hipFree(film_all); film_all = nullptr; film_all_bytes = 0; }
      const hipError_t e = hipMalloc(reinterpret_cast<void**>(&film_all), need);
      if (e != hipSuccess) { film_all = nullptr; return k22_set_error_hip(e, __FILE__, __LINE__); }
      film_all_bytes = need;
    }
    lr->film = film_all;
    lr->temb = lr->film + rows_all * film_total;
    lr->e1 = lr->temb + rows_all * tw.mc;
    lr->emb = lr->e1 + rows_all * tw.ted;
    return K22_OK;
  }
  int loop_prologue(const LoopRows& lr, const float* timesteps, int n_calls, const float* inpaint_image, const float* inpaint_mask, hipStream_t s) {
    if (lr.hoist) {
      const int spl = 8 / B;
      for (int k0 = 0; k0 < n_calls; k0 += spl) {
        const int rows = (n_calls - k0 < spl ? n_calls - k0 : spl) * B;
        const int64_t r0 = (int64_t)k0 * B;
        const int rc = time_rows(timesteps + r0, lr.temb + r0 * tw.mc, lr.e1 + r0 * tw.ted, lr.emb + r0 * tw.ted, lr.film + r0 * film_total, rows, s);
        if (rc) return rc;
      }
    }
    if (cfg.in_channels == 9) {
      const size_t pb = (size_t)B, hw = (size_t)H * W;
      if (int rc = copy_d2d(ptr(s_img), inpaint_image, pb * 4 * hw * 4, s)) return rc;
      if (int rc = copy_d2d(ptr(s_mask), inpaint_mask, pb * hw * 4, s)) return rc;
    }
    return K22_OK;
  }
  int loop_model(const LoopRows& lr, const float* cur, const float* timesteps, int call, hipStream_t s) {
    const size_t half = (size_t)(B / 2) * 4 * H * W * sizeof(float);
    if (int rc = copy_d2d(ptr(s_xin), cur, half, s)) return rc;
    if (int rc = copy_d2d(ptr(s_xin) + half, cur, half, s)) return rc;
    if (lr.hoist) {
      film_cur = lr.film + (int64_t)call * B * film_total;
    } else {
      if (int rc = copy_d2d(ptr(s_t), timesteps + (size_t)call * B, (size_t)B * 4, s)) return rc;
    }
    return exec(s);
  }
  template <typename F> int loop_run(const std::vector<unsigned long long>& key, const float* timesteps, const float* inpaint_image,
                                     const float* inpaint_mask, int use_graph, hipStream_t st, F body) {
    auto run_loop = [&](hipStream_t s) -> int { const int rc = body(s); film_cur = nullptr; return rc; };
    if (!use_graph) {
      const int rc = run_loop(st);
      if (rc == K22_OK) loop_count_launch();
      return rc;
    }
    if (!loop || key != loop_key) {
      if (!warmed) {
        const size_t pb = (size_t)B, hw = (size_t)H * W;
        hipError_t e = hipMemsetAsync(ptr(s_xin), 0, pb * 4 * hw * 4, st);
        if (e != hipSuccess) return k22_set_error_hip(e, __FILE__, __LINE__);
        if (int rc = copy_d2d(ptr(s_t), timesteps, pb * 4, st)) return rc;
        if (cfg.in_channels == 9) {
          if (int rc = copy_d2d(ptr(s_img), inpaint_image, pb * 4 * hw * 4, st)) return rc;
          if (int rc = copy_d2d(ptr(s_mask), inpaint_mask, pb * hw * 4, st)) return rc;
        }
        if (int rc = exec_eager(st)) return rc;
        e = hipStreamSynchronize(st);
        if (e != hipSuccess) return k22_set_error_hip(e, __FILE__, __LINE__);
      }
      if (int rc = loop.capture(cap, run_loop)) return rc;
      loop_key = key;
      loop_count_capture();
    }
    const int rc = loop.launch(st);
    if (rc == K22_OK) loop_count_launch();
    return rc;
  }

  int run_ops_range(hipStream_t st, size_t lo, size_t hi) {
    for (size_t i = lo; i < hi && i < ops.size(); ++i) { int rc = ops[i](st); if (rc) return rc; }
    return K22_OK;
  }
  int run_ops(hipStream_t st) { return run_ops_range(st, 0, ops.size()); }

  void op_gn(OpList& L, const Act& in, const std::string& pfx, int64_t film_off,
             int act, int mode, int pad, Slot* dst, const GnLink* link = nullptr) {
    const int Bn = B, C = in.C(), HW = in.H * in.W;
    const int nsplit = gn_nsplit(Bn, HW);
    const bool fused = in.st0 != nullptr && (in.s1 == nullptr || in.st1 != nullptr);
    if (!fused) need(s_part, (size_t)Bn * nsplit * C * 2 * sizeof(float));
    need(s_coeff, (size_t)Bn * C * 2 * sizeof(float));
    const int Ho = mode == 1 ? in.H / 2 : (mode == 2 ? in.H * 2 : in.H);
    const int Wo = mode == 1 ? in.W / 2 : (mode == 2 ? in.W * 2 : in.W);
    need(dst, (size_t)Bn * (Ho + 2 * pad) * (Wo + 2 * pad) * C * esz);
    const float* gamma = Wf(pfx + ".weight");
    const float* beta = Wf(pfx + ".bias");
    const Act a = in;
    const int dt = sdt;
    const int x3 = k22_is_split(dtype) ? 1 : 0;
    const double gn_bytes = (double)Bn * HW * C * esz * (fused ? 1.0 : 2.0) + (double)Bn * (Ho + 2 * pad) * (Wo + 2 * pad) * C * esz;
    L.push_back(Op([=](hipStream_t st) {
      const void* x0 = ptr(a.s0);
      const void* x1 = a.s1 ? ptr(a.s1) : nullptr;
      GnCoeffParams cp = {};
      if (fused) {
        cp.src[0].st = ptr<float>(a.st0); cp.src[0].rpi = a.p0->rpi; cp.src[0].C = a.C0;
        if (a.s1) { cp.src[1].st = ptr<float>(a.st1); cp.src[1].rpi = a.p1->rpi; cp.src[1].C = a.C1; }
        if (cp.src[0].rpi <= 0 || (a.s1 && cp.src[1].rpi <= 0)) return k22_set_error(K22_EINVAL, "unet: producer delivered no GroupNorm partial sums");
      } else {
        GnStatsParams sp;
        sp.x0 = x0; sp.x1 = x1; sp.C0 = a.C0; sp.C1 = a.C1;
        sp.HW = HW; sp.B = Bn; sp.groups = 32; sp.nsplit = nsplit; sp.partial = ptr<float>(s_part);
        int rc = launch_gn_stats(sp, dt, st);
        if (rc) return rc;
        cp.src[0].st = ptr<float>(s_part); cp.src[0].rpi = nsplit; cp.src[0].C = C;
      }
      cp.HW = HW; cp.C = C; cp.groups = 32; cp.eps = 1e-5f;
      cp.gamma = gamma; cp.beta = beta;
      cp.film = film_off >= 0 ? film_base() + film_off : nullptr; cp.film_ld = film_total;
      cp.coeff = ptr<float>(s_coeff);
      GnApplyParams ap = {};
      ap.x0 = x0; ap.x1 = x1; ap.C0 = a.C0; ap.C1 = a.C1; ap.B = Bn; ap.H = a.H; ap.W = a.W;
      ap.mode = mode; ap.pad = pad; ap.act = act; ap.coeff = ptr<float>(s_coeff); ap.out = ptr(dst); ap.out_x3 = x3;
      int rc = launch_gn_coeff(cp, Bn, st);
      if (rc) return rc;
      if (link != nullptr && link->consumer != nullptr && conv3_algo_fuses_gn(link->consumer->cfg.algo)) return K22_OK;
      return launch_gn_apply(ap, dt, st);
    }, OP_GN, 0.0, gn_bytes, fused ? 2 : 3));
  }

  static void apply_cfg(IgemmParams& q, const Cfg& c) { tuned_apply_cfg(q, c); }
  int op_dt(const Tuned& t) const { return t.dt >= 0 ? t.dt : dtype; }
  void make_candidates(Tuned& t) { tuned_make_candidates(t, op_dt(t)); }
  void default_cfg(Tuned& t) { tuned_default_cfg(t, op_dt(t)); }
  void finish_cfg(Tuned& t) { tuned_finish_cfg(t, op_dt(t)); }
  size_t max_splitk_bytes(const Tuned& t) const { return tuned_max_splitk_bytes(t, op_dt(t), autotune != 0); }
  int max_rpi(const Tuned& t) const { return tuned_max_rpi(t, op_dt(t), autotune != 0); }

  int x2_plan = 0;
  enum ConvRole { CONV_IN = 0, CONV_OUT = 1, CONV_HEAD = 2 };
  int conv_dt(int role, int Hc) const {
    if (dtype != K22_F16X2) return dtype;
    if (role == CONV_HEAD) return K22_F16X3;
    if (Hc >= H) return (x2_plan >> role) & 1 ? K22_F16X2 : K22_F16X3;
    return K22_F16X2;
  }
  int gemm_dt(bool qkv) const { return dtype == K22_F16X2 ? (qkv ? K22_F16X2 : K22_F16X3) : dtype; }

  Tuned* op_conv(OpList& L, int role, Slot* src, int Hc, int Wc, int Cin, int Cout,
                 const std::string& pfx, const Act* residual, Slot* dst, int out_mode, Slot* stats = nullptr,
                 const Act* skip_in = nullptr, const std::string& skip_pfx = std::string(), const Act* gn_in = nullptr, int gn_act = K22_ACT_NONE) {
    tuned.emplace_back();
    Tuned* t = &tuned.back();
    t->dt = conv_dt(role, Hc);
    IgemmParams& p = t->p;
    p = igemm_conv3_problem(B, Hc, Wc, Cin, Cout, out_mode);
    p.Wp = W_(pfx + ".weight"); p.bias = Wf(pfx + ".bias");
    Act sk;
    if (skip_in) {
      sk = *skip_in;
      p.S0 = reinterpret_cast<const void*>(1); p.S1 = sk.s1 ? reinterpret_cast<const void*>(1) : nullptr;
      p.SK0 = sk.C0; p.SK1 = sk.C1;
      p.Ws = W_(skip_pfx + ".weight"); p.bias2 = Wf(skip_pfx + ".bias");
    }
    t->want_stats = stats != nullptr;
    Slot *wf = nullptr, *wsf = nullptr;
    if (stream_frag && k22_esz(dtype) == 2 && p.M <= 1152 && (stream_supported(p, dtype, 5) || stream_supported(p, dtype, 9))) {
      wf = new_slot();
      need(wf, stream_frag_bytes(p.Npad, 9, Cin, dtype));
      frag_jobs.push_back({p.Wp, wf, p.Npad, 9, Cin});
      p.Wfrag = reinterpret_cast<const void*>(1);
      if (skip_in) {
        wsf = new_slot();
        need(wsf, stream_frag_bytes(p.Npad, 1, p.SK0 + p.SK1, dtype));
        frag_jobs.push_back({p.Ws, wsf, p.Npad, 1, p.SK0 + p.SK1});
        p.Wsfrag = reinterpret_cast<const void*>(1);
      }
    }
    make_candidates(*t);
    default_cfg(*t);
    if (wf && t->cfg.algo != IG_ALGO_STREAM && (t->from_table || !autotune)) {
      wf->bytes = 0; wf = nullptr;
      if (wsf) { wsf->bytes = 0; wsf = nullptr; frag_jobs.pop_back(); }
      frag_jobs.pop_back();
      p.Wfrag = nullptr; p.Wsfrag = nullptr;
      make_candidates(*t);
      default_cfg(*t);
    }
    need(s_splitk, max_splitk_bytes(*t));
    if (t->want_stats) need(stats, (size_t)B * max_rpi(*t) * Cout * 2 * sizeof(float));
// ... 152 lines not shown
  bool has_attn(int ds) const {
    for (int i = 0; i < cfg.n_attention_ds; ++i) if (cfg.attention_ds[i] == ds) return true;
    return false;
  }

  int plan(int nB, int nH, int nW) {
    const int n_down = cfg.n_levels - 1;
    if (nB < 1 || nH < 1 || nW < 1) return k22_set_error(K22_EINVAL, "unet: B, H, W must be positive");
    if (nH % (1 << n_down) || nW % (1 << n_down)) return k22_set_error(K22_EINVAL, "unet: H, W must be divisible by 2^(levels-1)");
    if (nB > 8) return k22_set_error(K22_EINVAL, "unet: batch (2*bs) must be <= 8 per engine call");
    begin_plan();
    B = nB; H = nH; W = nW;
    gn_links.clear();
    ops.clear(); cond_ops.clear(); hint_ops.clear(); s_ctxkv.clear(); frag_jobs.clear(); frag_done = false; n_attn = 0;
    cond_set = false; hint_set = false;
    loop.drop();
    const int mc = cfg.model_channels, ted = 4 * mc;

    film_total = 0;
    {
      int ch = mc * cfg.channel_mult[0];
      for (int l = 0; l < cfg.n_levels; ++l) {
        for (int i = 0; i < cfg.num_res_blocks; ++i) { ch = mc * cfg.channel_mult[l]; film_total += 2 * ch; }
        if (l != cfg.n_levels - 1) film_total += 2 * ch;
      }
      film_total += 2 * 2 * ch;
      for (int l = cfg.n_levels - 1; l >= 0; --l)
        for (int i = 0; i <= cfg.num_res_blocks; ++i) {
          ch = mc * cfg.channel_mult[l];
          film_total += 2 * ch;
          if (l && i == cfg.num_res_blocks) film_total += 2 * ch;
        }
    }

    s_xin = new_slot((size_t)B * 4 * H * W * 4); s_img = new_slot((size_t)B * 4 * H * W * 4);
    s_mask = new_slot((size_t)B * H * W * 4); s_t = new_slot((size_t)B * 4 + 64);
    s_out = new_slot((size_t)B * cfg.out_channels * H * W * 4);
    s_temb = new_slot((size_t)B * mc * 4); s_e1 = new_slot((size_t)B * ted * 4); s_emb = new_slot((size_t)B * ted * 4);
    s_film = new_slot((size_t)B * film_total * 4); s_xfproj = new_slot((size_t)B * ted * 4);
    s_ctx = new_slot((size_t)B * cfg.ctx_len * cfg.ctx_dim * esz);
    const int ntext_p = cfg.ctx_len - cfg.n_image_embs;
    s_full = new_slot((size_t)B * (ntext_p > 0 ? ntext_p : 1) * cfg.text_dim1 * 4); s_pool = new_slot((size_t)B * cfg.text_dim2 * 4);
    s_imgemb = new_slot((size_t)B * cfg.image_dim * 4);
    s_tmpf = new_slot((size_t)B * cfg.n_image_embs * cfg.ctx_dim * 4 + (size_t)B * ted * 4);
    s_tmpf2 = new_slot((size_t)B * ted * 4);
    s_fullT = new_slot((size_t)B * (ntext_p > 0 ? ntext_p : 1) * cfg.text_dim1 * esz);
    s_ctxf = new_slot(cfg.head_type == 1 ? (size_t)B * cfg.ctx_len * cfg.ctx_dim * 4 : 0);
    if (cfg.hint_channels) {
      s_hint = new_slot((size_t)B * 4 * H * W * 4);
      s_hintin = new_slot((size_t)B * cfg.hint_channels * 64 * H * W * 4);
      for (int i = 0; i < 2; ++i) s_hbuf[i] = new_slot((size_t)B * 16 * 64 * H * W * 4);
    }
    s_part = new_slot(); s_coeff = new_slot(); s_P1 = new_slot(); s_U1 = new_slot(); s_P2 = new_slot(); s_S = new_slot();
    s_N = new_slot(); s_QKV = new_slot(); s_KALL = new_slot(); s_VT = new_slot(); s_ATT = new_slot();
    s_splitk = new_slot(256);
    s_U1st = new_slot();
    s_flush = new_slot(autotune ? ((size_t)320 << 20) : 0);
    for (int i = 0; i < 3; ++i) { s_h[i] = new_slot(); s_hst[i] = new_slot(); }
    int hrot = 0, hcur = 0;
    auto next_h = [&]() { hcur = hrot; hrot = (hrot + 1) % 3; return s_h[hcur]; };
    auto cur_hst = [&]() { return s_hst[hcur]; };

    if (cfg.head_type == 1) build_cond_ops_22(); else build_cond_ops();
    if (cfg.hint_channels) build_hint_ops();

    {
      tw.freqs = Wf("time_freqs");
      tw.w0 = Wf("time_embed.0.weight"); tw.b0 = Wf("time_embed.0.bias");
      tw.w2 = Wf("time_embed.2.weight"); tw.b2 = Wf("time_embed.2.bias");
      tw.we = W_("emb_layers.weight"); tw.be = Wf("emb_layers.bias");
      tw.mc = mc; tw.ted = ted; tw.dt = sdt;
      const int Bn = B;
      ops.push_back([=](hipStream_t st) {
        if (film_cur) return (int)K22_OK;
        return time_rows(ptr<float>(s_t), ptr<float>(s_temb), ptr<float>(s_e1), ptr<float>(s_emb), ptr<float>(s_film), Bn, st);
      });
    }

    int64_t film_cursor = 0;
    std::vector<Act> hs;
    int ch = mc * cfg.channel_mult[0];
    {
      Slot* d = new_slot((size_t)B * H * W * ch * esz);
      ConvInParams cp = {};
      cp.w = Wf("input_blocks.0.0.weight"); cp.bias = Wf("input_blocks.0.0.bias");
      cp.B = B; cp.H = H; cp.W = W; cp.Cin = cfg.in_channels; cp.Cout = ch;
      const int dt = sdt; const bool inpaint = cfg.in_channels == 9, hinted = cfg.in_channels == 8;
      const int premul = (hinted || cfg.head_type == 1) ? 1 : 0;
      ops.push_back([=](hipStream_t st) {
        ConvInParams q = cp;
        q.x = ptr<float>(s_xin); q.img = inpaint ? ptr<float>(s_img) : (hinted ? ptr<float>(s_hint) : nullptr);
        q.mask = inpaint ? ptr<float>(s_mask) : nullptr; q.img_premul = premul;
        q.out = ptr(d);
        return launch_conv_in(q, dt, st);
      });
      Act a; a.s0 = d; a.C0 = ch; a.H = H; a.W = W;
      hs.push_back(a);
    }
    Act h = hs.back();
    int ds = 1, blk = 1;
    for (int l = 0; l < cfg.n_levels; ++l) {
      for (int i = 0; i < cfg.num_res_blocks; ++i) {
        const int co = mc * cfg.channel_mult[l];
        const std::string pfx = "input_blocks." + std::to_string(blk);
        Slot* d = new_slot();
        if (has_attn(ds)) {
          Slot* rd = next_h();
          Act r = resblock(pfx + ".0", h, co, 0, film_cursor, rd, cur_hst());
          h = attnblock(pfx + ".1", r, d, new_slot());
        } else {
          h = resblock(pfx + ".0", h, co, 0, film_cursor, d, new_slot());
        }
        ch = co; hs.push_back(h); ++blk;
      }
      if (l != cfg.n_levels - 1) {
        const std::string pfx = "input_blocks." + std::to_string(blk);
        Slot* d = new_slot();
        h = resblock(pfx + ".0", h, ch, 1, film_cursor, d, new_slot());
        hs.push_back(h); ++blk; ds *= 2;
      }
    }
    {
      Slot* d0 = next_h(); Slot* st0 = cur_hst();
      Act r = resblock("middle_block.0", h, ch, 0, film_cursor, d0, st0);
      Slot* da = next_h(); Slot* sta = cur_hst();
      Act a = attnblock("middle_block.1", r, da, sta);
      Slot* d2 = next_h(); Slot* st2 = cur_hst();
      h = resblock("middle_block.2", a, ch, 0, film_cursor, d2, st2);
    }
    blk = 0;
    for (int l = cfg.n_levels - 1; l >= 0; --l) {
      for (int i = 0; i <= cfg.num_res_blocks; ++i) {
        const Act skip = hs.back(); hs.pop_back();
        Act cat; cat.s0 = h.s0; cat.C0 = h.C0; cat.s1 = skip.s0; cat.C1 = skip.C0; cat.H = h.H; cat.W = h.W;
        cat.p0 = h.p0; cat.st0 = h.st0; cat.p1 = skip.p0; cat.st1 = skip.st0;
        if (skip.H != h.H || skip.W != h.W) return k22_set_error(K22_EINVAL, "unet: skip shape mismatch");
        const int co = mc * cfg.channel_mult[l];
        const std::string pfx = "output_blocks." + std::to_string(blk);
        { Slot* d = next_h(); Slot* dst_st = cur_hst(); h = resblock(pfx + ".0", cat, co, 0, film_cursor, d, dst_st); }
        int sub = 1;
        if (has_attn(ds)) { Slot* da = next_h(); Slot* sta = cur_hst(); h = attnblock(pfx + "." + std::to_string(sub), h, da, sta); ++sub; }
        if (l && i == cfg.num_res_blocks) {
          { Slot* d = next_h(); Slot* dst_st = cur_hst(); h = resblock(pfx + "." + std::to_string(sub), h, co, 2, film_cursor, d, dst_st); }
          ds /= 2;
        }
        ch = co; ++blk;
      }
    }
    if (film_cursor != film_total) return k22_set_error(K22_EINVAL, "unet: internal FiLM width mismatch");
    op_gn(ops, h, "out.0", -1, K22_ACT_SILU, 0, 1, s_P1);
    op_conv(ops, CONV_HEAD, s_P1, H, W, ch, cfg.out_channels, "out.2", nullptr, s_out, IG_OUT_NCHW_F32);

    return finish_plan();
  }

  void build_cond_ops_22() {
    const int mc = cfg.model_channels, ted = 4 * mc, Bn = B, dt = sdt;
    const int cd = cfg.ctx_dim, S = cfg.ctx_len, di = cfg.image_dim;
    const float* w_cp = Wf("head22.ctx_proj.weight"); const float* b_cp = Wf("head22.ctx_proj.bias");
    const float* g_cn = Wf("head22.ctx_norm.weight"); const float* b_cn = Wf("head22.ctx_norm.bias");
    const float* w_ep = Wf("head22.emb_proj.weight"); const float* b_ep = Wf("head22.emb_proj.bias");
    const float* g_en = Wf("head22.emb_norm.weight"); const float* b_en = Wf("head22.emb_norm.bias");
    cond_ops.push_back([=](hipStream_t st) {
      float* proj = ptr<float>(s_tmpf);
      float* embp = ptr<float>(s_tmpf) + (size_t)Bn * S * cd;
      LinearSmallParams lp = {};
      lp.x = ptr<float>(s_imgemb); lp.ldx = di; lp.W = w_cp; lp.bias = b_cp; lp.out = proj; lp.ldo = S * cd;
      lp.M = Bn; lp.N = S * cd; lp.K = di;
      int rc = launch_linear_smallm(lp, K22_F32, st);
      if (rc) return rc;
      rc = launch_layernorm_f32(proj, g_cn, b_cn, ptr<float>(s_ctxf), Bn * S, cd, 1e-5f, st);
      if (rc) return rc;
      rc = launch_cast_rows(ptr<float>(s_ctxf), ptr(s_ctx), Bn * S, cd, cd, cd, dt, st);
      if (rc) return rc;
      lp.W = w_ep; lp.bias = b_ep; lp.out = embp; lp.ldo = ted; lp.N = ted;
      rc = launch_linear_smallm(lp, K22_F32, st);
      if (rc) return rc;
      return launch_layernorm_f32(embp, g_en, b_en, ptr<float>(s_xfproj), Bn, ted, 1e-5f, st);
    });
  }

  void build_hint_ops() {
    static const int chans[9] = {0, 16, 16, 32, 32, 96, 96, 256, 4};
    static const int strides[8] = {1, 1, 2, 1, 2, 1, 2, 1};
    int hin = 8 * H, win = 8 * W, cin = cfg.hint_channels;
    for (int k = 0; k < 8; ++k) {
      const float* w = Wf("hint." + std::to_string(k) + ".weight");
      const float* b = Wf("hint." + std::to_string(k) + ".bias");
      const int cout = chans[k + 1], stride = strides[k], Bn = B, ci = cin, hi = hin, wi = win;
      Slot* src = k == 0 ? s_hintin : s_hbuf[(k - 1) & 1];
      Slot* dst = k == 7 ? s_hint : s_hbuf[k & 1];
      hint_ops.push_back([=](hipStream_t st) {
        ConvDirectParams q = {};
        q.x = ptr<float>(src); q.w = w; q.bias = b; q.y = ptr<float>(dst);
        q.B = Bn; q.Cin = ci; q.Cout = cout; q.Hin = hi; q.Win = wi; q.stride = stride; q.act = k == 7 ? K22_ACT_NONE : K22_ACT_SILU;
        return launch_conv3x3_direct(q, st);
      });
      cin = cout;
      if (stride == 2) { hin = (hin - 1) / 2 + 1; win = (win - 1) / 2 + 1; }
    }
  }

  void build_cond_ops() {
    const int mc = cfg.model_channels, ted = 4 * mc, Bn = B, dt = sdt;
    const int nie = cfg.n_image_embs, cd = cfg.ctx_dim, S = cfg.ctx_len, ntext = S - nie;
    const float* w_cs = Wf("clip_to_seq.weight"); const float* b_cs = Wf("clip_to_seq.bias");
    const float* w_pn = Wf("proj_n.weight"); const float* b_pn = Wf("proj_n.bias");
    const float* g_ln = Wf("ln_model_n.weight"); const float* b_ln = Wf("ln_model_n.bias");
    const float* w_il = Wf("img_layer.weight"); const float* b_il = Wf("img_layer.bias");
    const int d1 = cfg.text_dim1, d2 = cfg.text_dim2, di = cfg.image_dim;
    cond_ops.push_back([=](hipStream_t st) {
      float* clipseq = ptr<float>(s_tmpf);
      float* proj = ptr<float>(s_tmpf) + (size_t)Bn * nie * cd;
      LinearSmallParams lp = {};
      lp.x = ptr<float>(s_imgemb); lp.ldx = di; lp.W = w_cs; lp.bias = b_cs; lp.out = clipseq; lp.ldo = nie * cd;
      lp.M = Bn; lp.N = nie * cd; lp.K = di;
      int rc = launch_linear_smallm(lp, K22_F32, st);
      if (rc) return rc;
// ... 294 lines not shown
```

### kandinsky-2_amd/csrc/igemm.hip

```cpp
#include "kernels.h"
#include <stdlib.h>
#include <type_traits>

template <int N> __device__ __forceinline__ void wait_vmcnt() { asm volatile("s_waitcnt vmcnt(%0)" ::"n"(N) : "memory"); }

template <typename T> __device__ __forceinline__ void store4(T* dst, const float* v);
template <> __device__ __forceinline__ void store4<bf16_t>(bf16_t* dst, const float* v) {
  uint2 w;
  w.x = pack2_bf16(v[0], v[1]);
  w.y = pack2_bf16(v[2], v[3]);
  *reinterpret_cast<uint2*>(dst) = w;
}
template <> __device__ __forceinline__ void store4<f16_t>(f16_t* dst, const float* v) {
  uint2 w;
  w.x = pack2_f16(v[0], v[1]);
  w.y = pack2_f16(v[2], v[3]);
  *reinterpret_cast<uint2*>(dst) = w;
}
template <> __device__ __forceinline__ void store4<float>(float* dst, const float* v) {
  *reinterpret_cast<float4*>(dst) = make_float4(v[0], v[1], v[2], v[3]);
}
template <> __device__ __forceinline__ void store4<x3_t>(x3_t* dst, const float* v) { store4<float>(reinterpret_cast<float*>(dst), v); }
template <> __device__ __forceinline__ void store4<x2_t>(x2_t* dst, const float* v) { store4<float>(reinterpret_cast<float*>(dst), v); }
template <typename T> __device__ __forceinline__ void load4f(const T* src, float* v);
// ... 337 lines not shown
    }
    v[0] = a.x; v[1] = a.y; v[2] = a.z; v[3] = a.w;
    if (p.bias != nullptr) {
      const float4 b = *reinterpret_cast<const float4*>(p.bias + n);
      v[0] += b.x; v[1] += b.y; v[2] += b.z; v[3] += b.w;
    }
    if (p.bias2 != nullptr) {
      const float4 b = *reinterpret_cast<const float4*>(p.bias2 + n);
      v[0] += b.x; v[1] += b.y; v[2] += b.z; v[3] += b.w;
    }
    if (res != nullptr) {
      float rv[4];
      if (p.res_f32) load4f<float>(reinterpret_cast<const float*>(p.residual) + (int64_t)m * p.ldr + n, rv);
      else load4f<T>(res + (int64_t)m * p.ldr + n, rv);
#pragma unroll
      for (int e = 0; e < 4; ++e) v[e] += rv[e];
    }
#pragma unroll
    for (int e = 0; e < 4; ++e) v[e] = apply_act(v[e], p.act);
    if (p.out_mode == IG_OUT_ROWMAJOR) {
      store4<T>(reinterpret_cast<T*>(p.out) + (int64_t)m * p.ldo + n, v);
#pragma unroll
      for (int e = 0; e < 4; ++e) v[e] = to_f32(from_f32<T>(v[e]));
    } else {
      store4<float>(reinterpret_cast<float*>(p.out) + (int64_t)m * p.ldo + n, v);
    }
  }
  if (p.stats == nullptr) return;
#pragma unroll
  for (int e = 0; e < 4; ++e) {
    red[r][cq * 4 + e][0] = ok ? v[e] : 0.f;
    red[r][cq * 4 + e][1] = ok ? v[e] * v[e] : 0.f;
  }
  __syncthreads();
  if (threadIdx.x < 128) {
    const int ch = threadIdx.x >> 1, which = threadIdx.x & 1;
    float a = 0.f;
#pragma unroll
    for (int rr = 0; rr < 16; ++rr) a += red[rr][ch][which];
    const int nn = blockIdx.y * 64 + ch;
    if (nn < p.N) p.stats[((int64_t)blockIdx.x * p.N + nn) * 2 + which] = a;
  }
}

static IgemmOptions g_opts;
void igemm_set_default_stages(int v) { g_opts.stages = (v >= 2 && v <= 4) ? v : -1; }
void igemm_set_xcd_remap(int v) { g_opts.xcd_remap = v ? 1 : 0; }
void igemm_set_gemm_algo(int v) { g_opts.gemm_algo = (v == IG_ALGO_GEMM8 || v == IG_ALGO_STREAM) ? v : 0; }
void igemm_set_conv_algo(int v) {
  bool ok = v == IG_ALGO_GENERIC || v == IG_ALGO_STREAM || (igemm_algo_is_halo(v) && !igemm_algo_is_debug(v));
#ifdef K22_DEBUG_VARIANTS
  ok = ok || igemm_algo_is_debug(v);
#endif
  g_opts.conv_algo = ok ? v : 0;
}

static bool reduce_rows_ok(const IgemmParams& p, bool stats) {
  const int hw = (p.taps == 9 || stats) ? p.H * p.W : 0;
  return hw > 0 && hw % 16 == 0 && (p.N & 3) == 0 && (p.ldo & 3) == 0 && (p.ldr & 3) == 0 &&
         (p.out_mode == IG_OUT_ROWMAJOR || p.out_mode == IG_OUT_ROWMAJOR_F32);
}

int igemm_resolve(const IgemmParams& p, int dtype, IgemmLaunch* out) {
  const IgemmOptions o = g_opts;
  if (dtype < K22_BF16 || dtype > K22_F16X2) return k22_set_error(K22_EINVAL, "igemm: bad dtype");
  const int BK = k22_bk(dtype);
  const int nkt = p.taps * (p.Kc / BK);
  const bool qkv = p.out_mode == IG_OUT_QKV;
  IgemmLaunch L = {};
  L.xcd_remap = o.xcd_remap;
  L.block = 512;
  const int want = (p.stages < 2 && o.stages >= 0) ? o.stages : p.stages;
  auto blocks = [&](int bm, int bn) { return ((p.M + bm - 1) / bm) * ((p.N + bn - 1) / bn); };
  if (p.algo == IG_ALGO_STREAM || (p.algo == IG_ALGO_AUTO && (p.taps == 9 ? o.conv_algo : o.gemm_algo) == IG_ALGO_STREAM)) {
    const int mb = p.force_bm == 288 ? 9 : 5;
    if (stream_supported(p, dtype, mb)) {
      L.family = IG_FAM_STREAM; L.algo = IG_ALGO_STREAM; L.bm = mb * 32; L.bn = 64;
      const int nslab = p.Kc / 64, nb = stream_mtiles(p, mb);
      L.splitk = p.splitk > 0 ? p.splitk : (nb >= 240 ? 1 : 240 / nb);
      if (L.splitk > nslab) L.splitk = nslab;
      if (L.splitk < 1) L.splitk = 1;
      L.block = 256; L.grid = (unsigned)nb; L.lds = stream_lds_bytes(p, mb);
    }
  }
  const int conv_algo = (p.algo && p.algo != IG_ALGO_STREAM) ? p.algo : (o.conv_algo == IG_ALGO_STREAM ? 0 : o.conv_algo);
  if (!L.algo && p.taps == 9 && conv_algo != IG_ALGO_GENERIC && p.N >= 128 && !p.a_raw) {
    IgemmParams ph = p;
    ph.algo = igemm_algo_is_halo(conv_algo) ? conv_algo : IG_ALGO_HALO;
    int bm = 0;
    if (p.force_bm == 256 || p.force_bm == 128) {
      if (conv3_halo_supported(ph, dtype, p.force_bm) && (conv_algo >= IG_ALGO_HALO || p.force_bn == 0)) bm = p.force_bm;
    } else if (p.force_bm == 0) {
      if (conv3_halo_supported(ph, dtype, 256)) bm = 256;
      else if (conv3_halo_supported(ph, dtype, 128)) bm = 128;
    }
    if (bm) {
      L.algo = ph.algo; L.bm = bm; L.bn = 128;
      const int nslab = (p.Kc / BK) * (L.algo == IG_ALGO_HALO3 ? 2 : 1);
      const int nb = (p.M / (p.H * p.W)) * conv3_halo_tiles_per_image(p, bm) * ((p.N + 127) / 128);
      if (p.splitk > 0) {
        L.splitk = p.splitk;
      } else {
        int sk = 1;
        while (nb * sk < 200 && sk < 16 && (p.Kc / BK) / (sk * 2) >= 2) sk *= 2;
        L.splitk = sk;
      }
      if (L.splitk > nslab) L.splitk = nslab;
      if (L.splitk < 1) L.splitk = 1;
      L.grid = (unsigned)nb;
      L.depth = conv3_halo_ring(ph, bm);
      if (want >= 2 && want < L.depth) L.depth = want == 5 ? 4 : want;
      const bool split = k22_is_split(dtype);
      if (conv3_algo_fuses_gn(L.algo)) {
        L.family = IG_FAM_SPEC;
        L.pipe = (L.algo == IG_ALGO_SPEC_PIPE && !(bm == 256 && (dtype == K22_F16X3 || dtype == K22_F32))) ? 1 : 0;
      } else if (split) {
        if (igemm_algo_is_debug(L.algo)) return k22_set_error(K22_EINVAL, "conv3_halo: no measurement-only variants in split precision");
        L.family = IG_FAM_HALO; L.pipe = 2;
      } else if (L.algo == IG_ALGO_HALO3) {
        L.family = IG_FAM_HALO3;
      } else if (igemm_algo_is_debug(L.algo)) {
#ifdef K22_DEBUG_VARIANTS
        if (L.algo == IG_ALGO_DBG_SPEC_NO_DMA || L.algo == IG_ALGO_DBG_SPEC_NO_WAIT) {
          if (dtype != K22_BF16 || bm != 256) return k22_set_error(K22_EINVAL, "conv3_halo: the debug variants are bf16, BM = 256 only");
          L.family = IG_FAM_SPEC; L.pipe = 1; L.dbg = L.algo == IG_ALGO_DBG_SPEC_NO_DMA ? 1 : 2; L.depth = L.depth == 2 ? 2 : 4;
        } else {
          if (dtype != K22_BF16 || bm != 256) return k22_set_error(K22_EINVAL, "conv3_halo: debug variants are bf16, BM = 256 only");
          L.family = IG_FAM_HALO; L.pipe = L.algo == IG_ALGO_DBG_NO_DMA ? 3 : 4;
        }
#else
        return k22_set_error(K22_EINVAL, "conv3_halo: measurement-only variants need a -DK22_DEBUG_VARIANTS build");
#endif
      } else {
        L.family = IG_FAM_HALO;
        L.pipe = L.algo == IG_ALGO_HALO_PIPE ? 1 : (L.algo == IG_ALGO_HALO_ASM ? 2 : 0);
      }
      L.lds = conv3_halo_lds_bytes(ph, bm, L.depth);
    }
  }
  if (!L.algo && p.taps == 1 && (p.algo == IG_ALGO_GEMM8 || (p.algo == IG_ALGO_AUTO && o.gemm_algo == IG_ALGO_GEMM8))) {
    const int hw = p.H > 0 ? p.H * p.W : p.M;
    int bm = 0;
    if (p.force_bm == 256 || p.force_bm == 128) { if (gemm8_supported(p, dtype, p.force_bm)) bm = p.force_bm; }
    else if (gemm8_supported(p, dtype, 256))
      bm = ((p.M / hw) * ((hw + 255) / 256) * ((p.N + 127) / 128) >= 400 || hw % 256 == 0) ? 256 : 128;
    if (bm) {
      L.algo = IG_ALGO_GEMM8; L.bm = bm; L.bn = 128;
      L.splitk = p.splitk > 0 ? p.splitk : 1;
      if (qkv) L.splitk = 1;
      if (L.splitk > p.Kc / BK) L.splitk = p.Kc / BK;
      L.grid = (unsigned)((p.M / hw) * gemm8_tiles_per_image(p, bm) * ((p.N + 127) / 128));
      if ((want == 3 || want == 4) && gemm8_spec_supported(dtype)) {
        L.family = IG_FAM_GEMM8_SPEC; L.pipe = 1;
        L.depth = (want == 4 && bm == 128) ? 2 : (bm == 256 ? 3 : 4);
      } else {
        L.family = IG_FAM_GEMM8;
        L.depth = bm == 256 ? 3 : (want == 2 ? 2 : 4);
        L.a_raw = (k22_is_split(dtype) && p.a_raw) ? 1 : 0;
      }
      L.lds = gemm8_lds_bytes(bm, L.depth);
    }
  }
  if (!L.algo) {
    L.family = IG_FAM_GENERIC; L.algo = IG_ALGO_GENERIC; L.block = 256;
    if (p.force_bm && p.force_bn) { L.bm = p.force_bm; L.bn = p.force_bn; }
    else if (p.N <= 64) { L.bm = (p.M >= 128) ? 128 : 64; L.bn = 64; }
    else if (blocks(128, 128) >= 160) { L.bm = 128; L.bn = 128; }
    else if (p.M > 64) { L.bm = 128; L.bn = 64; }
    else { L.bm = 64; L.bn = 64; }
    if ((L.bm != 128 && L.bm != 64) || (L.bn != 128 && L.bn != 64)) return k22_set_error(K22_EINVAL, "igemm: unsupported tile configuration");
    L.grid = (unsigned)blocks(L.bm, L.bn);
    if (p.splitk > 0) {
      L.splitk = p.splitk;
    } else {
      int sk = 1;
      while ((int)L.grid * sk < 200 && sk < 16 && nkt / (sk * 2) >= 6) sk *= 2;
      L.splitk = sk;
    }
    if (L.splitk > nkt) L.splitk = nkt > 0 ? nkt : 1;
    static const int env_stages = [] { const char* e = getenv("K22_IGEMM_STAGES"); const int v = e ? atoi(e) : 2; return (v < 2 || v > 4) ? 2 : v; }();
    L.depth = (p.stages >= 2 && p.stages <= 4) ? p.stages : (o.stages >= 0 ? o.stages : env_stages);
    L.a_raw = (k22_is_split(dtype) && p.a_raw) ? 1 : 0;
    static const int dbg_pad = getenv("K22_DBG_LDS_PAD") ? atoi(getenv("K22_DBG_LDS_PAD")) : 0;
    const size_t smem0 = (size_t)L.depth * (L.bm + L.bn) * 128;
    L.lds = dbg_pad == 1 ? (smem0 + 1279) / 1280 * 1280 : (dbg_pad == 2 ? smem0 + 4096 : smem0);
  }
  const bool stream = L.family == IG_FAM_STREAM, generic = L.family == IG_FAM_GENERIC;
  if (qkv && !stream) {
    if (p.splitk > 1) return k22_set_error(K22_EINVAL, "igemm: the qkv projection splits K only on the streaming kernel");
    L.splitk = 1;
  }
  if (!stream) {
    if (p.res_f32 && !generic) return k22_set_error(K22_EINVAL, "igemm: fp32 residual is not supported by the halo kernel");
    if (p.gn_coeff != nullptr && !conv3_algo_fuses_gn(L.algo))
      return k22_set_error(K22_EINVAL, "igemm: the fused GroupNorm-apply input needs the specialised halo kernel (algo 11 / 12)");
    if (p.S0 != nullptr && generic) return k22_set_error(K22_EINVAL, "igemm: the fused 1x1 skip connection needs the halo kernel");
    if (p.stats != nullptr && L.splitk == 1 && generic)
      return k22_set_error(K22_EINVAL, "igemm: GroupNorm partial sums requested from a configuration that cannot produce them");
  }
  L.grid *= (unsigned)L.splitk;
  const bool finishes = stream || L.splitk > 1;
  L.finish = !finishes ? IG_FINISH_NONE : (reduce_rows_ok(p, p.stats != nullptr) ? IG_FINISH_ROWS : IG_FINISH_FLAT);
  if (p.taps == 1 && (generic || p.H <= 0 || qkv)) L.stats_rows_per_image = 0;
  else if (finishes) L.stats_rows_per_image = reduce_rows_ok(p, true) ? p.H * p.W / 16 : 0;
  else if (generic) L.stats_rows_per_image = 0;
  else L.stats_rows_per_image = p.taps == 1 ? gemm8_tiles_per_image(p, L.bm) : conv3_halo_tiles_per_image(p, L.bm);
  *out = L;
  return K22_OK;
}

int igemm_choose_splitk(const IgemmParams& p, int dtype) {
  IgemmParams q = p;
  q.splitk = 0;
  IgemmLaunch L;
  return igemm_resolve(q, dtype, &L) == K22_OK ? L.splitk : 1;
}

int igemm_stats_rows_per_image(const IgemmParams& p, int dtype) {
  IgemmLaunch L;
  return igemm_resolve(p, dtype, &L) == K22_OK ? L.stats_rows_per_image : 0;
}

static int launch_finish(const IgemmParams& q, int dtype, const IgemmLaunch& L, hipStream_t stream) {
  return k22_with_dtype(dtype, [&](auto tag) {
    using T0 = typename decltype(tag)::type;
    using T = typename std::conditional<is_x3<T0>::value, float, T0>::type;
    if (L.finish == IG_FINISH_ROWS) {
      hipLaunchKernelGGL((splitk_reduce_rows_kernel<T>), dim3((q.M + 15) / 16, (q.N + 63) / 64), dim3(256), 0, stream, q);
    } else {
      const int64_t total = (int64_t)q.M * q.N;
      int nb = (int)((total / 4 + 255) / 256);
      if (nb > 2048) nb = 2048;
      if (nb < 1) nb = 1;
      hipLaunchKernelGGL((splitk_reduce_kernel<T>), dim3(nb), dim3(256), 0, stream, q);
    }
    K22_CHECK_LAUNCH();
    return (int)K22_OK;
  });
}

template <typename T, int BM, int BN, int STAGES, bool ARAW>
static int run_generic(const IgemmParams& q, const IgemmLaunch& L, hipStream_t stream) {
  static LdsAttrGuard guard;
  return launch_lds_kernel(igemm_kernel<T, BM, BN, STAGES, ARAW>, guard, L.grid, L.block, L.lds, (int)L.lds, stream, q);
}
template <typename T, int BM, int BN>
static int launch_generic_tile(const IgemmParams& q, const IgemmLaunch& L, hipStream_t stream) {
  auto depth = [&](auto araw) {
    constexpr bool ARAW = decltype(araw)::value;
    if (L.depth == 2) return run_generic<T, BM, BN, 2, ARAW>(q, L, stream);
    if (L.depth == 3) return run_generic<T, BM, BN, 3, ARAW>(q, L, stream);
    return run_generic<T, BM, BN, 4, ARAW>(q, L, stream);
  };
  if constexpr (is_x3<T>::value) { if (L.a_raw) return depth(std::true_type{}); }
  return depth(std::false_type{});
}
static int launch_generic(const IgemmParams& q, int dtype, const IgemmLaunch& L, hipStream_t stream) {
  return k22_with_dtype(dtype, [&](auto tag) {
    using T = typename decltype(tag)::type;
    if (L.bm == 128) return L.bn == 128 ? launch_generic_tile<T, 128, 128>(q, L, stream) : launch_generic_tile<T, 128, 64>(q, L, stream);
    return L.bn == 128 ? launch_generic_tile<T, 64, 128>(q, L, stream) : launch_generic_tile<T, 64, 64>(q, L, stream);
  });
}

int launch_igemm(const IgemmParams& p, int dtype, hipStream_t stream) {
  const int BK = k22_bk(dtype);
  if (p.a_raw && !k22_is_split(dtype)) return k22_set_error(K22_EINVAL, "igemm: a_raw is an option of the split-precision arithmetics only");
  if (p.M <= 0 || p.N <= 0) return K22_OK;
  if (p.taps != 1 && p.taps != 9) return k22_set_error(K22_EINVAL, "igemm: taps must be 1 or 9");
  if (p.Kc % BK != 0 || p.K0 % BK != 0) return k22_set_error(K22_EINVAL, "igemm: K per tap must be a multiple of 64 (bf16) / 32 (fp32)");
  if (p.Npad % 64 != 0 || p.Npad < p.N) return k22_set_error(K22_EINVAL, "igemm: Npad must be roundup(N,64)");
  if (p.K0 < p.Kc && p.A1 == nullptr) return k22_set_error(K22_EINVAL, "igemm: A1 missing for concat operand");
  if (p.out_mode == IG_OUT_QKV) {
    if (p.taps != 1 || p.N % 192 || (p.ldo & 3) || !p.kall || !p.vtall || p.att_T <= 0 || p.M % p.att_T || p.residual)
      return k22_set_error(K22_EINVAL, "igemm: bad qkv-projection problem (N = 3*heads*64, no residual)");
  }
  IgemmParams q = p;
  IgemmLaunch L;
  if (int rc = igemm_resolve(q, dtype, &L)) return rc;
  if (L.family == IG_FAM_STREAM) {
    if (p.partial == nullptr) return k22_set_error(K22_EINVAL, "igemm: the streaming kernel needs the fp32 partial buffer");
  } else if (L.splitk > 1 && p.partial == nullptr) {
    q.splitk = 1;
    if (int rc = igemm_resolve(q, dtype, &L)) return rc;
  }
  if (L.finish == IG_FINISH_FLAT && q.stats != nullptr)
    return k22_set_error(K22_EINVAL, "igemm: GroupNorm partial sums are not available for this split-K problem");
  q.splitk = L.splitk; q.xcd_remap = L.xcd_remap; q.algo = L.algo;
  int rc;
  switch (L.family) {
    case IG_FAM_STREAM: rc = launch_stream(q, dtype, L, stream); break;
    case IG_FAM_GEMM8: case IG_FAM_GEMM8_SPEC: rc = launch_gemm8(q, dtype, L, stream); break;
    case IG_FAM_SPEC: rc = launch_conv3_halo_spec(q, dtype, L, stream); break;
    case IG_FAM_GENERIC: rc = launch_generic(q, dtype, L, stream); break;
    default: rc = launch_conv3_halo(q, dtype, L, stream); break;
  }
  if (rc || L.finish == IG_FINISH_NONE) return rc;
  return launch_finish(q, dtype, L, stream);
}
```

### kandinsky-2_amd/csrc/kernels.h

```cpp
#pragma once
#include "common.h"

#include <atomic>
#include <type_traits>

#define K22_OK 0
#define K22_EINVAL (-1)
#define K22_EHIP (-2)
#define K22_ENOMEM (-3)

struct LdsAttrGuard { std::atomic<unsigned long long> done{0}; };
inline int k22_ensure_lds_attr(LdsAttrGuard& g, const void* fn, int bytes, const char* file, int line) {
  int dev = 0;
  (void)hipGetDevice(&dev);
  const unsigned long long bit = 1ull << (dev & 63);
  if (g.done.load(std::memory_order_acquire) & bit) return K22_OK;
  const hipError_t e = hipFuncSetAttribute(fn, hipFuncAttributeMaxDynamicSharedMemorySize, bytes);
  if (e != hipSuccess) return k22_set_error_hip(e, file, line);
  g.done.fetch_or(bit, std::memory_order_release);
  return K22_OK;
}

enum IgemmOut { IG_OUT_ROWMAJOR = 0,
                IG_OUT_ROWMAJOR_F32 = 1,
                IG_OUT_NCHW_F32 = 2,
                IG_OUT_QKV = 3 };

struct IgemmParams {
  const void* A0;
  const void* A1;
  const void* Wp;
  const float* bias;
  const void* residual;
  void* out;
  float* partial;
  int M, N, Npad;
  int Kc;
  int K0;
  int taps;
  int H, W;
  long lda0, lda1;
  int ldo, ldr;
  int out_mode;
  int act;
  int splitk;
  int force_bm, force_bn;
  int stages = -1;
  int xcd_remap;
  int algo;
  const void* S0; const void* S1; const void* Ws; const float* bias2;
  int SK0, SK1;
  void* kall; void* vtall;
  int att_T, att_S, att_Tkp;
  unsigned long long* trace;
  int res_f32;
  float* stats;
  const void* Wfrag; const void* Wsfrag;
  int a_raw;
  const float* gn_coeff; const void* gn_x0; const void* gn_x1; int gn_C0, gn_act;
  unsigned long long* st_trace;
  int st_tm, st_rb, st_mtiles, st_buf;
};
static_assert(sizeof(IgemmParams) == 320 && std::is_trivially_copyable<IgemmParams>::value, "IgemmParams layout");

enum IgemmAlgo {
  IG_ALGO_AUTO = 0,
  IG_ALGO_GENERIC = 1,
  IG_ALGO_HALO = 2,
  IG_ALGO_HALO3 = 3,
  IG_ALGO_HALO_PIPE = 6,
  IG_ALGO_HALO_ASM = 7,
  IG_ALGO_DBG_NO_DMA = 8,
  IG_ALGO_DBG_NO_MFMA = 9,
  IG_ALGO_GEMM8 = 10,
  IG_ALGO_SPEC = 11,
  IG_ALGO_SPEC_PIPE = 12,
  IG_ALGO_DBG_SPEC_NO_DMA = 13,
  IG_ALGO_DBG_SPEC_NO_WAIT = 14,
  IG_ALGO_STREAM = 20
};
struct IgemmAlgoName { int algo; const char* name; };
constexpr IgemmAlgoName IGEMM_ALGO_NAMES[] = {{IG_ALGO_GENERIC, "gen"},   {IG_ALGO_HALO, "halo"},   {IG_ALGO_HALO3, "hal3"}, {IG_ALGO_HALO_PIPE, "hal6"},
                                              {IG_ALGO_HALO_ASM, "hal7"}, {IG_ALGO_GEMM8, "gem8"}, {IG_ALGO_SPEC, "spec"},  {IG_ALGO_SPEC_PIPE, "spcp"}};
inline const char* igemm_algo_name(int algo) {
  for (const IgemmAlgoName& a : IGEMM_ALGO_NAMES) if (a.algo == algo) return a.name;
  return "auto";
}
inline bool igemm_algo_is_halo(int a) { return a == IG_ALGO_HALO || a == IG_ALGO_HALO3 || (a >= IG_ALGO_HALO_PIPE && a <= IG_ALGO_DBG_NO_MFMA) || (a >= IG_ALGO_SPEC && a <= IG_ALGO_DBG_SPEC_NO_WAIT); }
inline bool igemm_algo_is_debug(int a) { return a == IG_ALGO_DBG_NO_DMA || a == IG_ALGO_DBG_NO_MFMA || a == IG_ALGO_DBG_SPEC_NO_DMA || a == IG_ALGO_DBG_SPEC_NO_WAIT; }

inline IgemmParams igemm_gemm_problem(int M, int N, int K0, int K1, int out_mode = IG_OUT_ROWMAJOR, int act = 0) {
  IgemmParams p = {};
  p.M = M; p.N = N; p.Npad = (N + 63) / 64 * 64; p.Kc = K0 + K1; p.K0 = K0; p.taps = 1;
  p.lda0 = K0; p.lda1 = K1; p.ldo = N; p.ldr = N; p.out_mode = out_mode; p.act = act;
  return p;
}
inline IgemmParams igemm_conv3_problem(int B, int H, int W, int Cin, int Cout, int out_mode = IG_OUT_ROWMAJOR, int act = 0) {
  IgemmParams p = {};
  p.M = B * H * W; p.N = Cout; p.Npad = (Cout + 63) / 64 * 64; p.Kc = Cin; p.K0 = Cin; p.taps = 9; p.H = H; p.W = W;
  p.ldo = Cout; p.ldr = Cout; p.out_mode = out_mode; p.act = act;
  return p;
}

enum IgemmFamily { IG_FAM_GENERIC, IG_FAM_HALO, IG_FAM_HALO3, IG_FAM_SPEC, IG_FAM_GEMM8, IG_FAM_GEMM8_SPEC, IG_FAM_STREAM };
enum IgemmFinish { IG_FINISH_NONE, IG_FINISH_FLAT, IG_FINISH_ROWS };
struct IgemmLaunch {
  int family;
  int algo;
  int bm, bn;
  int splitk;
  int depth;
  int pipe;
  int dbg;
  int a_raw;
  int xcd_remap;
  int finish;
  int stats_rows_per_image;
  unsigned grid, block;
  size_t lds;
};
struct IgemmOptions { int conv_algo = 0, gemm_algo = 0, stages = -1, xcd_remap = 1; };
int igemm_resolve(const IgemmParams& p, int dtype, IgemmLaunch* L);

template <typename K>
inline int launch_lds_kernel(K kernel, LdsAttrGuard& guard, unsigned grid, unsigned block, size_t smem, int attr_bytes, hipStream_t stream, const IgemmParams& params) {
  if (int rc = k22_ensure_lds_attr(guard, reinterpret_cast<const void*>(kernel), attr_bytes, __FILE__, __LINE__)) return rc;
  hipLaunchKernelGGL(kernel, dim3(grid), dim3(block), smem, stream, params);
  K22_CHECK_LAUNCH();
  return K22_OK;
}

struct IgemmStatsInfo { int rows_per_image; };
int igemm_stats_rows_per_image(const IgemmParams& p, int dtype);

int launch_igemm(const IgemmParams& p, int dtype, hipStream_t stream);

bool conv3_halo_supported(const IgemmParams& p, int dtype, int bm);
inline bool conv3_algo_fuses_gn(int algo) { return algo == IG_ALGO_SPEC || algo == IG_ALGO_SPEC_PIPE; }
int conv3_halo_tiles_per_image(const IgemmParams& p, int bm);
int conv3_halo_ring(const IgemmParams& p, int bm);
size_t conv3_halo_lds_bytes(const IgemmParams& p, int bm, int depth);
int launch_conv3_halo(const IgemmParams& p, int dtype, const IgemmLaunch& L, hipStream_t stream);
int launch_conv3_halo_spec(const IgemmParams& p, int dtype, const IgemmLaunch& L, hipStream_t stream);
int launch_conv3_halo_trace(const IgemmParams& p, int dtype, hipStream_t stream);
bool gemm8_supported(const IgemmParams& p, int dtype, int bm);
bool gemm8_spec_supported(int dtype);
int gemm8_tiles_per_image(const IgemmParams& p, int bm);
size_t gemm8_lds_bytes(int bm, int depth);
int launch_gemm8(const IgemmParams& p, int dtype, const IgemmLaunch& L, hipStream_t stream);
bool stream_supported(const IgemmParams& p, int dtype, int mb);
int stream_mtiles(const IgemmParams& p, int mb);
size_t stream_lds_bytes(const IgemmParams& p, int mb);
int launch_stream(const IgemmParams& p, int dtype, const IgemmLaunch& L, hipStream_t stream);
long stream_launch_count();
long loop_capture_count();
long loop_launch_count();
size_t stream_frag_bytes(int Npad, int taps, int Kc, int dtype);
int launch_stream_repack(const void* W, void* out, int Npad, int taps, int Kc, int dtype, hipStream_t stream);
void igemm_set_gemm_algo(int v);
void igemm_set_conv_algo(int v);
void igemm_set_default_stages(int v);
void igemm_set_xcd_remap(int v);
void attention_set_pipe(int v);
int igemm_choose_splitk(const IgemmParams& p, int dtype);
```

### kandinsky-2_amd/csrc/tuning.h

```cpp
#pragma once
#include "kernels.h"

#include <deque>
#include <functional>
#include <map>
#include <mutex>
#include <string>
#include <tuple>
#include <vector>
#include <stdio.h>
#include <stdlib.h>

struct Cfg { int algo = 0, bm = 0, bn = 0, splitk = 0, stages = 0; };

struct TunedSlot;

typedef std::tuple<int, int, int, int, int, int, int, int, int, bool> TileKey;
struct TileTable {
  std::map<TileKey, std::pair<Cfg, float>> m;
  std::mutex mu;
  bool env_loaded = false;
  size_t measured = 0;
};
inline TileTable& tile_table() { static TileTable t; return t; }
// ... 33 lines not shown
  return (int)tt.m.size();
}
inline void tile_table_load_env_once() {
  TileTable& tt = tile_table();
  bool need;
  { std::lock_guard<std::mutex> lk(tt.mu); need = !tt.env_loaded; tt.env_loaded = true; }
  if (need) if (const char* cp = getenv("K22_TUNE_CACHE")) (void)tile_table_load_file(cp);
}

struct Tuned {
  IgemmParams p = {};
  std::vector<Cfg> cands;
  Cfg cfg;
  bool want_stats = false;
  int rpi = 0;
  float best_us = 0.f;
  bool from_table = false;
  int dt = -1;
  void* aux0 = nullptr; void* aux1 = nullptr;
  std::function<int(hipStream_t)> run;
};

inline void tuned_apply_cfg(IgemmParams& q, const Cfg& c) {
  q.algo = c.algo; q.force_bm = c.bm; q.force_bn = c.bn; q.splitk = c.splitk; q.stages = c.stages;
}

inline void tuned_make_candidates(Tuned& t, int dtype) {
  const IgemmParams& p = t.p;
  const int BK = k22_bk(dtype);
  const int nkt = p.taps * (p.Kc / BK);
  std::vector<Cfg> all;
  if (p.taps == 9) {
    const int B = p.M / (p.H * p.W);
    for (int algo : {IG_ALGO_HALO, IG_ALGO_HALO_ASM, IG_ALGO_HALO_PIPE, IG_ALGO_HALO3, IG_ALGO_SPEC, IG_ALGO_SPEC_PIPE}) {
      if (algo == IG_ALGO_HALO3 && p.H > 16) continue;
      if (k22_is_split(dtype) && (algo == IG_ALGO_HALO || algo == IG_ALGO_HALO_PIPE)) continue;
      IgemmParams ph = p;
      ph.algo = algo;
      const int nsplit_max = (p.Kc / BK) * (algo == IG_ALGO_HALO3 ? 2 : 1);
      for (int bm : {256, 128}) {
        if (!conv3_halo_supported(ph, dtype, bm) || p.N < 128) continue;
        const int nb = B * conv3_halo_tiles_per_image(p, bm) * ((p.N + 127) / 128);
        for (int sk : {1, 2, 3, 4, 5, 6, 8, 10, 12}) {
          if (sk > nsplit_max || (sk > 1 && nb * sk > 800) || (sk > 1 && nb >= 256)) continue;
          Cfg c; c.algo = algo; c.bm = bm; c.bn = 0; c.splitk = sk; c.stages = 0;
          all.push_back(c);
        }
      }
    }
  }
  if (p.taps == 1) {
    const int hw = p.H > 0 ? p.H * p.W : p.M;
    for (int bm : {256, 128}) {
      IgemmParams q = p;
      q.algo = IG_ALGO_GEMM8; q.force_bm = bm;
      if (!gemm8_supported(q, dtype, bm)) continue;
      const int nb = (p.M / hw) * gemm8_tiles_per_image(p, bm) * ((p.N + 127) / 128);
      for (int sk : {1, 2, 3, 4, 6}) {
        if (sk > 1 && (nkt / sk < 4 || nb * sk > 800 || nb >= 256 || p.out_mode == IG_OUT_QKV)) continue;
        for (int stg : {0, 2, 3, 4}) {
          if ((stg == 2 || stg == 4) && bm != 128) continue;
          if (stg >= 3 && !gemm8_spec_supported(dtype)) continue;
          Cfg c; c.algo = IG_ALGO_GEMM8; c.bm = bm; c.bn = 0; c.splitk = sk; c.stages = stg;
          all.push_back(c);
        }
      }
    }
  }
  if (k22_esz(dtype) == 2 && p.Wfrag != nullptr && p.taps == 9) {
    for (int mb : {5, 9}) {
      IgemmParams q = p;
      q.algo = IG_ALGO_STREAM; q.force_bm = mb * 32;
      if (!stream_supported(q, dtype, mb)) continue;
      const int nb = stream_mtiles(q, mb);
      if (nb > 320) continue;
      const int nslab = p.Kc / 64;
      for (int sk : {1, 2, 3, 4, 5, 6, 8, 10, 12, 16}) {
        if (sk > nslab || (sk > 1 && nb * sk > 320)) continue;
        Cfg c; c.algo = IG_ALGO_STREAM; c.bm = mb * 32; c.bn = 0; c.splitk = sk; c.stages = 0;
        all.push_back(c);
      }
    }
  }
  const int tiles[3][2] = {{128, 128}, {128, 64}, {64, 64}};
  const bool skinny = p.taps == 1;
  for (auto& tl : tiles) {
    if (p.S0 != nullptr) break;
    if (tl[1] == 128 && p.N <= 64) continue;
    if (tl[0] == 128 && p.M <= 64) continue;
    const int nb = ((p.M + tl[0] - 1) / tl[0]) * ((p.N + tl[1] - 1) / tl[1]);
    for (int sk : {1, 2, 4, 8, 16}) {
      if (sk > 1 && (nkt / sk < 4 || nb * sk > 1536 || nb >= 384 || p.out_mode == IG_OUT_QKV)) continue;
      for (int stg : {2, 3, 4}) {
        if (stg > 2 && !skinny) continue;
        if (stg * (tl[0] + tl[1]) * 128 > 160 * 1024) continue;
        Cfg c; c.algo = IG_ALGO_GENERIC; c.bm = tl[0]; c.bn = tl[1]; c.splitk = sk; c.stages = stg;
        all.push_back(c);
      }
    }
  }
  t.cands.clear();
  for (auto& c : all) {
    IgemmParams q = p;
    tuned_apply_cfg(q, c);
    if ((size_t)c.splitk * p.M * p.N * sizeof(float) > ((size_t)96 << 20) && c.splitk > 1) continue;
    if (t.want_stats && igemm_stats_rows_per_image(q, dtype) <= 0) continue;
    t.cands.push_back(c);
  }
}

inline TileKey tuned_key(const Tuned& t, int dtype) {
  const IgemmParams& p = t.p;
  if (dtype == K22_F16) dtype = K22_BF16;
  return TileKey(dtype, p.taps, p.M, p.N, p.Kc, p.K0 + (p.S0 ? 100000 * (p.SK0 + p.SK1) : 0), p.H, p.W,
                 p.out_mode + 16 * p.res_f32 + 32 * p.act + 256 * p.a_raw, t.want_stats);
}

inline bool tuned_is_candidate(const Tuned& t, const Cfg& c) {
  for (auto& k : t.cands)
    if (k.algo == c.algo && k.bm == c.bm && k.bn == c.bn && k.splitk == c.splitk && (k.stages == c.stages || (c.algo >= IG_ALGO_HALO && c.algo != IG_ALGO_GEMM8))) return true;
  return false;
}

inline bool tile_table_lookup(const Tuned& t, int dtype, Cfg* out, float* us) {
  tile_table_load_env_once();
  TileTable& tt = tile_table();
  std::lock_guard<std::mutex> lk(tt.mu);
  auto it = tt.m.find(tuned_key(t, dtype));
  static const bool x2_own = getenv("K22_X2_OWN_LINES") && atoi(getenv("K22_X2_OWN_LINES")) != 0;
  if ((it == tt.m.end() || !tuned_is_candidate(t, it->second.first)) && dtype == K22_F16X2 && !x2_own) it = tt.m.find(tuned_key(t, K22_F16X3));
  if (it == tt.m.end() || !tuned_is_candidate(t, it->second.first)) return false;
  *out = it->second.first;
  if (us) *us = it->second.second * 1e3f;
  return true;
}

inline void tuned_finish_cfg(Tuned& t, int dtype) {
  IgemmParams q = t.p;
  tuned_apply_cfg(q, t.cfg);
  t.rpi = t.want_stats ? igemm_stats_rows_per_image(q, dtype) : 0;
}

inline void tuned_default_cfg(Tuned& t, int dtype) {
  IgemmParams q = t.p;
  q.algo = 0; q.force_bm = 0; q.force_bn = 0; q.splitk = 0; q.stages = 0;
  Cfg c; c.algo = 0; c.bm = 0; c.bn = 0; c.splitk = igemm_choose_splitk(q, dtype); c.stages = 0;
  if (q.out_mode == IG_OUT_QKV) c.splitk = 1;
  tuned_apply_cfg(q, c);
  if (t.want_stats && igemm_stats_rows_per_image(q, dtype) <= 0) {
    if (t.cands.empty()) { t.want_stats = false; }
    else c = t.cands[0];
  }
  t.cfg = c;
  t.from_table = false;
  if (t.p.M >= 64 && t.cands.size() >= 2) {
    Cfg tc; float us = 0.f;
    if (tile_table_lookup(t, dtype, &tc, &us)) { t.cfg = tc; t.best_us = us; t.from_table = true; }
  }
  tuned_finish_cfg(t, dtype);
}

inline size_t tuned_max_splitk_bytes(const Tuned& t, int dtype, bool autotune) {
  size_t m = 0;
  auto upd = [&](const Cfg& c) {
    IgemmParams q = t.p;
    tuned_apply_cfg(q, c);
// ... 84 lines not shown
```

Measured before the change: 148.3 steps/s.

## Add small-N output conv kernel and fuse GroupNorm stats into stem conv

Adds an MFMA-based 3x3 convolution kernel specialised for very small output channel counts (N<=8, the UNet out conv) with weights held in LDS, and registers it as a tuning candidate. The stem conv_in kernel now reads the latent directly with a batch period, which removes the two per-step device copies that duplicated x for CFG. It also writes GroupNorm partial sums so the first block's GroupNorm skips a separate stats pass. In exchange the code gains complexity and new kernels whose tile choice depends on the autotuner.

```diff
diff --git a/include/k22.h b/include/k22.h
--- a/include/k22.h
+++ b/include/k22.h
@@ -118,6 +118,13 @@
 int k22_conv3x3_gnstats(const void* x_padded, const void* Wp, const float* bias, const void* residual, void* out,
                         void* partial, int B, int H, int W, int Cin, int Cout, int Npad, int splitk, int bm, int bn,
                         float* stats, int stats_capacity_rows, int* rows_per_image, int dtype, void* stream);
+int k22_conv3x3_smalln(const void* x_padded, const void* Wp, const float* bias, const void* residual, float* out, int B, int H, int W, int Cin,
+                       int Cout, int Npad, int dtype, void* stream);
+int k22_conv_in(const float* x, const float* img, const float* mask, const float* w, const float* bias, void* out, int B, int H, int W,
+                int Cin, int Cout, int img_premul, int period, float* sums, int sums_capacity_rows, int* rows_per_image, int dtype,
+                void* stream);
+int k22_conv_in_reference(const float* x, const float* img, const float* mask, const float* w, const float* bias, void* out, int B, int H,
+                          int W, int Cin, int Cout, int img_premul, int dtype, void* stream);
 int k22_gemm_gnstats(const void* A, const void* Wp, const float* bias, const void* residual, void* out, void* partial,
                      int B, int H, int W, int N, int Npad, int K, int splitk, int bm, float* stats,
                      int stats_capacity_rows, int* rows_per_image, int dtype, void* stream);
diff --git a/kandinsky-2_amd/_lib.py b/kandinsky-2_amd/_lib.py
--- a/kandinsky-2_amd/_lib.py
+++ b/kandinsky-2_amd/_lib.py
@@ -129,6 +129,9 @@
     "k22_conv3x3": (_I, [_P, _P, _P, _P, _P, _P, _I, _I, _I, _I, _I, _I, _I, _I, _I, _I, _I, _I, _P]),
     "k22_conv3x3_skip": (_I, [_P, _P, _P, _P, _P, _I, _I, _P, _P, _P, _P, _I, _I, _I, _I, _I, _I, _I, _I, _I, _P]),
     "k22_gemm_gnstats": (_I, [_P, _P, _P, _P, _P, _P, _I, _I, _I, _I, _I, _I, _I, _I, _P, _I, C.POINTER(_I), _I, _P]),
+    "k22_conv3x3_smalln": (_I, [_P, _P, _P, _P, _P, _I, _I, _I, _I, _I, _I, _I, _P]),
+    "k22_conv_in": (_I, [_P, _P, _P, _P, _P, _P, _I, _I, _I, _I, _I, _I, _I, _P, _I, C.POINTER(_I), _I, _P]),
+    "k22_conv_in_reference": (_I, [_P, _P, _P, _P, _P, _P, _I, _I, _I, _I, _I, _I, _I, _P]),
     "k22_conv3x3_gnstats": (_I, [_P, _P, _P, _P, _P, _P, _I, _I, _I, _I, _I, _I, _I, _I, _I, _P, _I, C.POINTER(_I), _I, _P]),
     "k22_igemm_cfg_accepted": (_I, [C.POINTER(K22IgemmProblem)]),
     "k22_igemm_cfg": (_I, [C.POINTER(K22IgemmProblem), C.POINTER(K22IgemmOperands), C.POINTER(_I), _P]),
diff --git a/kandinsky-2_amd/csrc/capi.hip b/kandinsky-2_amd/csrc/capi.hip
--- a/kandinsky-2_amd/csrc/capi.hip
+++ b/kandinsky-2_amd/csrc/capi.hip
@@ -82,6 +82,7 @@
   if (name && !strcmp(name, "stream_launches")) return stream_launch_count();
   if (name && !strcmp(name, "loop_captures")) return loop_capture_count();
   if (name && !strcmp(name, "loop_launches")) return loop_launch_count();
+  if (name && !strcmp(name, "gn_stats_launches")) return gn_stats_launch_count();
   return -1;
 }
 
@@ -184,6 +185,45 @@
   p.stats = stats;
   K22_DBG_FRAG(p);
   return launch_igemm(p, dtype, reinterpret_cast<hipStream_t>(stream));
+}
+
+int k22_conv3x3_smalln(const void* x_padded, const void* Wp, const float* bias, const void* residual, float* out, int B, int H, int W, int Cin,
+                       int Cout, int Npad, int dtype, void* stream) {
+  if (!x_padded || !Wp || !out) return k22_set_error(K22_EINVAL, "conv3x3_smalln: null argument");
+  if (B < 1 || H < 1 || W < 1) return k22_set_error(K22_EINVAL, "conv3x3_smalln: B, H, W must be positive");
+  IgemmParams p = igemm_conv3_problem(B, H, W, Cin, Cout, IG_OUT_NCHW_F32);
+  p.A0 = x_padded; p.Wp = Wp; p.bias = bias; p.residual = residual; p.out = out;
+  p.Npad = Npad; p.splitk = 1; p.algo = IG_ALGO_SMALLN;
+  return launch_igemm(p, dtype, reinterpret_cast<hipStream_t>(stream));
+}
+
+int k22_conv_in(const float* x, const float* img, const float* mask, const float* w, const float* bias, void* out, int B, int H, int W,
+                int Cin, int Cout, int img_premul, int period, float* sums, int sums_capacity_rows, int* rows_per_image, int dtype,
+                void* stream) {
+  const int rpi = conv_in_rows_per_image(H, W);
+  if (rows_per_image) *rows_per_image = rpi;
+  if (!x || !w || !bias || !out) return k22_set_error(K22_EINVAL, "conv_in: null argument");
+  if (!k22_dtype_ok(dtype)) return k22_set_error(K22_EINVAL, "conv_in: dtype must be a storage type (bf16, fp16, fp32)");
+  if (Cin > 4 && !img) return k22_set_error(K22_EINVAL, "conv_in: channels 4-7 need img");
+  if ((Cin == 9 || (Cin == 8 && !img_premul)) && !mask) return k22_set_error(K22_EINVAL, "conv_in: mask missing");
+  if (sums && (long)rpi * B > sums_capacity_rows) return k22_set_error(K22_ENOMEM, "conv_in: sums buffer too small");
+  ConvInParams p = {};
+  p.x = x; p.img = img; p.mask = mask; p.w = w; p.bias = bias; p.out = out;
+  p.B = B; p.H = H; p.W = W; p.Cin = Cin; p.Cout = Cout; p.img_premul = img_premul ? 1 : 0; p.period = period; p.sums = sums;
+  return launch_conv_in(p, dtype, reinterpret_cast<hipStream_t>(stream));
+}
+
+int k22_conv_in_reference(const float* x, const float* img, const float* mask, const float* w, const float* bias, void* out, int B, int H,
+                          int W, int Cin, int Cout, int img_premul, int dtype, void* stream) {
+  if (!x || !w || !bias || !out) return k22_set_error(K22_EINVAL, "conv_in_reference: null argument");
+  if (!k22_dtype_ok(dtype)) return k22_set_error(K22_EINVAL, "conv_in_reference: dtype must be a storage type (bf16, fp16, fp32)");
+  if (B < 1 || H < 1 || W < 1 || Cout < 1 || H > 65535 || B > 65535) return k22_set_error(K22_EINVAL, "conv_in_reference: bad shape");
+  if (Cin > 4 && !img) return k22_set_error(K22_EINVAL, "conv_in_reference: channels 4-7 need img");
+  if ((Cin == 9 || (Cin == 8 && !img_premul)) && !mask) return k22_set_error(K22_EINVAL, "conv_in_reference: mask missing");
+  ConvInParams p = {};
+  p.x = x; p.img = img; p.mask = mask; p.w = w; p.bias = bias; p.out = out;
+  p.B = B; p.H = H; p.W = W; p.Cin = Cin; p.Cout = Cout; p.img_premul = img_premul ? 1 : 0; p.period = B;
+  return launch_conv_in_reference(p, dtype, reinterpret_cast<hipStream_t>(stream));
 }
 
 int k22_gemm_gnstats(const void* A, const void* Wp, const float* bias, const void* residual, void* out, void* partial,
diff --git a/kandinsky-2_amd/csrc/conv3_smalln.hip b/kandinsky-2_amd/csrc/conv3_smalln.hip
--- /dev/null
+++ b/kandinsky-2_amd/csrc/conv3_smalln.hip
@@ -0,0 +1,108 @@
+#include "kernels.h"
+
+template <typename T> __device__ __forceinline__ f32x4_t mfma16(const u32x4_t a, const u32x4_t b, const f32x4_t c);
+template <> __device__ __forceinline__ f32x4_t mfma16<bf16_t>(const u32x4_t a, const u32x4_t b, const f32x4_t c) {
+  return __builtin_amdgcn_mfma_f32_16x16x32_bf16(__builtin_bit_cast(bf16x8_t, a), __builtin_bit_cast(bf16x8_t, b), c, 0, 0, 0);
+}
+template <> __device__ __forceinline__ f32x4_t mfma16<f16_t>(const u32x4_t a, const u32x4_t b, const f32x4_t c) {
+  return __builtin_amdgcn_mfma_f32_16x16x32_f16(__builtin_bit_cast(f16x8_t, a), __builtin_bit_cast(f16x8_t, b), c, 0, 0, 0);
+}
+
+constexpr int SMALLN_ROWS = 8, SMALLN_WAVES = 8, SMALLN_PIX = 16;
+
+template <typename T, int NKS>
+__global__ __launch_bounds__(64 * SMALLN_WAVES) void conv3_smalln_kernel(IgemmParams p) {
+  extern __shared__ __attribute__((aligned(16))) char smalln_smem[];
+  constexpr int Kc = NKS * 32;
+  constexpr int NKC = 9 * Kc / 8;
+  const int tid = threadIdx.x, lane = tid & 63, wave = tid >> 6;
+  constexpr int TOT = NKC * SMALLN_ROWS, NIT = (TOT + 64 * SMALLN_WAVES - 1) / (64 * SMALLN_WAVES);
+  u32x4_t wreg[NIT];
+  {
+    const T* Wg = reinterpret_cast<const T*>(p.Wp);
+#pragma unroll
+    for (int it = 0; it < NIT; ++it) {
+      const int i = tid + it * 64 * SMALLN_WAVES, kc = i >> 3, n = i & 7;
+      if (i < TOT) wreg[it] = *reinterpret_cast<const u32x4_t*>(Wg + (int64_t)n * (9 * Kc) + kc * 8);
+    }
+  }
+  const int ntx = (p.W + SMALLN_PIX - 1) / SMALLN_PIX;
+  const int ntiles = (p.M / p.W) * ntx;
+  const int tile = blockIdx.x * SMALLN_WAVES + wave;
+  const bool live = tile < ntiles;
+  const int tt = live ? tile : 0;
+  const int xt = tt % ntx, by = tt / ntx, y = by % p.H, b = by / p.H;
+  const int px = lane & 15, kq = lane >> 4;
+  const int xx = xt * SMALLN_PIX + px;
+  const int xl = xx < p.W ? xx : p.W - 1;
+  const int Wp2 = p.W + 2;
+  const T* a = reinterpret_cast<const T*>(p.A0) + (((int64_t)b * (p.H + 2) + y) * Wp2 + xl) * Kc + kq * 8;
+  const char* wl = smalln_smem + (kq * SMALLN_ROWS + (px & 7)) * 16;
+
+  u32x4_t ring[3][9];
+  auto load_slab = [&](int ks, u32x4_t* dst) {
+#pragma unroll
+    for (int tap = 0; tap < 9; ++tap)
+      dst[tap] = *reinterpret_cast<const u32x4_t*>(a + ((int64_t)(tap / 3) * Wp2 + (tap % 3)) * Kc + ks * 32);
+  };
+  load_slab(0, ring[0]);
+  load_slab(1, ring[1]);
+#pragma unroll
+  for (int it = 0; it < NIT; ++it) {
+    const int i = tid + it * 64 * SMALLN_WAVES;
+    if (i < TOT) *reinterpret_cast<u32x4_t*>(smalln_smem + (size_t)i * 16) = wreg[it];
+  }
+  __syncthreads();
+  f32x4_t acc = {0.f, 0.f, 0.f, 0.f};
+#pragma unroll
+  for (int ks = 0; ks < NKS; ++ks) {
+    if (ks + 2 < NKS) load_slab(ks + 2, ring[(ks + 2) % 3]);
+#pragma unroll
+    for (int tap = 0; tap < 9; ++tap)
+      acc = mfma16<T>(*reinterpret_cast<const u32x4_t*>(wl + (size_t)(tap * NKS + ks) * 512), ring[ks % 3][tap], acc);
+  }
+  if (!live || xx >= p.W) return;
+  const int64_t m = ((int64_t)b * p.H + y) * p.W + xx;
+  const T* res = reinterpret_cast<const T*>(p.residual);
+  float* out = reinterpret_cast<float*>(p.out);
+#pragma unroll
+  for (int i = 0; i < 4; ++i) {
+    const int n = kq * 4 + i;
+    if (n < p.N) {
+      float v = acc[i];
+      if (p.bias != nullptr) v += p.bias[n];
+      if (res != nullptr) v += to_f32(res[m * p.ldr + n]);
+      out[(((int64_t)b * p.N + n) * p.H + y) * p.W + xx] = v;
+    }
+  }
+}
+
+bool conv3_smalln_supported(const IgemmParams& p, int dtype) {
+  if (dtype != K22_BF16 && dtype != K22_F16) return false;
+  if (p.taps != 9 || p.N < 1 || p.N > SMALLN_ROWS || p.Npad < SMALLN_ROWS || p.out_mode != IG_OUT_NCHW_F32) return false;
+  if (p.Kc != 128 && p.Kc != 256 && p.Kc != 384) return false;
+  if (p.K0 != p.Kc || p.H < 1 || p.W < 1 || p.M < 1 || p.M % (p.H * p.W)) return false;
+  return p.S0 == nullptr && p.gn_coeff == nullptr && !p.res_f32 && p.act == K22_ACT_NONE && !p.a_raw;
+}
+size_t conv3_smalln_lds_bytes(const IgemmParams& p) { return (size_t)9 * p.Kc * SMALLN_ROWS * 2; }
+unsigned conv3_smalln_grid(const IgemmParams& p) {
+  const int tiles = (p.M / p.W) * ((p.W + SMALLN_PIX - 1) / SMALLN_PIX);
+  return (unsigned)((tiles + SMALLN_WAVES - 1) / SMALLN_WAVES);
+}
+
+template <typename T, int NKS>
+static int run_smalln(const IgemmParams& p, const IgemmLaunch& L, hipStream_t stream) {
+  static LdsAttrGuard guard;
+  return launch_lds_kernel(conv3_smalln_kernel<T, NKS>, guard, L.grid, L.block, L.lds, (int)L.lds, stream, p);
+}
+template <typename T>
+static int launch_smalln_t(const IgemmParams& p, const IgemmLaunch& L, hipStream_t stream) {
+  if (p.Kc == 128) return run_smalln<T, 4>(p, L, stream);
+  if (p.Kc == 256) return run_smalln<T, 8>(p, L, stream);
+  return run_smalln<T, 12>(p, L, stream);
+}
+int launch_conv3_smalln(const IgemmParams& p, int dtype, const IgemmLaunch& L, hipStream_t stream) {
+  if (!conv3_smalln_supported(p, dtype)) return k22_set_error(K22_EINVAL, "conv3_smalln: problem not supported (16-bit, N <= 8, Kc 128 / 256 / 384, fp32 NCHW out)");
+  if (p.stats != nullptr) return k22_set_error(K22_EINVAL, "conv3_smalln: no GroupNorm partial sums");
+  return dtype == K22_BF16 ? launch_smalln_t<bf16_t>(p, L, stream) : launch_smalln_t<f16_t>(p, L, stream);
+}
diff --git a/kandinsky-2_amd/csrc/elementwise.h b/kandinsky-2_amd/csrc/elementwise.h
--- a/kandinsky-2_amd/csrc/elementwise.h
+++ b/kandinsky-2_amd/csrc/elementwise.h
@@ -30,7 +30,10 @@
   void* out;
   int B, H, W, Cin, Cout;
   int img_premul;
+  int period;
+  float* sums;
 };
+inline int conv_in_rows_per_image(int H, int ) { return H; }
 struct ConvDirectParams {
   const float* x; const float* w; const float* bias; float* y;
   int B, Cin, Cout, Hin, Win, stride, act;
@@ -109,6 +112,8 @@
 int launch_gn_apply(const GnApplyParams& p, int dtype, hipStream_t s);
 int launch_resample(const void* x, void* y, int B, int H, int W, int C, int mode, int dtype, hipStream_t s);
 int launch_conv_in(const ConvInParams& p, int dtype, hipStream_t s);
+int launch_conv_in_reference(const ConvInParams& p, int dtype, hipStream_t s);
+long gn_stats_launch_count();
 int launch_timestep_embedding(const float* t, const float* freqs, float* out, int B, int half, hipStream_t s);
 int launch_linear_smallm(const LinearSmallParams& p, int wdtype, hipStream_t s);
 int launch_layernorm_f32(const float* x, const float* g, const float* b, float* y, int rows, int D, float eps, hipStream_t s);
diff --git a/kandinsky-2_amd/csrc/elementwise.hip b/kandinsky-2_amd/csrc/elementwise.hip
--- a/kandinsky-2_amd/csrc/elementwise.hip
+++ b/kandinsky-2_amd/csrc/elementwise.hip
@@ -1,5 +1,6 @@
 #include "kernels.h"
 #include "elementwise.h"
+#include <atomic>
 
 __device__ __forceinline__ void load4(const bf16_t* p, float* f) {
   const uint2 r = *reinterpret_cast<const uint2*>(p);
@@ -259,9 +260,100 @@
   }
 }
 
+constexpr int CONV_IN_R = 12, CONV_IN_MAX_WAVES = 8;
+template <typename T> __device__ __forceinline__ void store2_stored(T* dst, float a, float b, float& va, float& vb) {
+  const uint32_t w = pack2<T>(a, b);
+  *reinterpret_cast<uint32_t*>(dst) = w;
+  unpack2<T>(w, va, vb);
+}
+template <> __device__ __forceinline__ void store2_stored<f16_t>(f16_t* dst, float a, float b, float& va, float& vb) {
+  const f16_t ha = (f16_t)a, hb = (f16_t)b;
+  const f16x2_t v = {ha, hb};
+  *reinterpret_cast<f16x2_t*>(dst) = v;
+  va = (float)ha; vb = (float)hb;
+}
+template <> __device__ __forceinline__ void store2_stored<float>(float* dst, float a, float b, float& va, float& vb) {
+  *reinterpret_cast<float2*>(dst) = make_float2(a, b);
+  va = a; vb = b;
+}
+template <typename T, int CIN>
+__global__ __launch_bounds__(64 * CONV_IN_MAX_WAVES) void conv_in_kernel(ConvInParams p) {
+  constexpr int R = CONV_IN_R;
+  extern __shared__ float conv_in_smem[];
+  const int tid = threadIdx.x, lane = tid & 63, wave = tid >> 6, nthr = blockDim.x, nw = nthr >> 6;
+  const int y = blockIdx.x, b = blockIdx.y, bx = b % p.period;
+  const int nrun = (p.W + R - 1) / R, PW = nrun * R + 2;
+  float* patch = conv_in_smem;
+  float* red = conv_in_smem + CIN * 3 * PW;
+  const int hw = p.H * p.W;
+  for (int i = tid; i < CIN * 3 * PW; i += nthr) {
+    const int c = i / (3 * PW), r = (i / PW) % 3, xx = i % PW;
+    const int yy = y + r - 1, xs = xx - 1;
+    float v = 0.f;
+    if (yy >= 0 && yy < p.H && xs >= 0 && xs < p.W) {
+      const int64_t o = (int64_t)yy * p.W + xs;
+      if (c < 4) v = p.x[((int64_t)bx * 4 + c) * hw + o];
+      else if (c < 8) v = p.img[((int64_t)b * 4 + (c - 4)) * hw + o] * (p.img_premul ? 1.f : p.mask[(int64_t)b * hw + o]);
+      else v = p.mask[(int64_t)b * hw + o];
+    }
+    patch[i] = v;
+  }
+  __syncthreads();
+  T* out = reinterpret_cast<T*>(p.out) + (int64_t)(b * p.H + y) * p.W * p.Cout;
+  for (int n = 2 * lane; n < p.Cout; n += 128) {
+    float2 w[CIN * 9];
+#pragma unroll
+    for (int k = 0; k < CIN * 9; ++k) w[k] = *reinterpret_cast<const float2*>(p.w + (int64_t)k * p.Cout + n);
+    const float2 bias = *reinterpret_cast<const float2*>(p.bias + n);
+    float s0 = 0.f, q0 = 0.f, s1 = 0.f, q1 = 0.f;
+    for (int run = wave; run < nrun; run += nw) {
+      const int x0 = run * R;
+      float a0[R], a1[R], row[R + 2];
+#pragma unroll
+      for (int px = 0; px < R; ++px) { a0[px] = bias.x; a1[px] = bias.y; }
+#pragma unroll
+      for (int c = 0; c < CIN; ++c)
+#pragma unroll
+        for (int r = 0; r < 3; ++r) {
+#pragma unroll
+          for (int i = 0; i < R + 2; ++i) row[i] = patch[(c * 3 + r) * PW + x0 + i];
+#pragma unroll
+          for (int q = 0; q < 3; ++q) {
+            if (c == CIN - 1 && r == 2 && q == 2) break;
+#pragma unroll
+            for (int px = 0; px < R; ++px) {
+              a0[px] += w[c * 9 + r * 3 + q].x * row[px + q];
+              a1[px] += w[c * 9 + r * 3 + q].y * row[px + q];
+            }
+          }
+#pragma unroll
+          for (int px = 0; px < R; px += 4)
+            asm volatile("" : "+v"(a0[px]), "+v"(a0[px + 1]), "+v"(a0[px + 2]), "+v"(a0[px + 3]),
+                              "+v"(a1[px]), "+v"(a1[px + 1]), "+v"(a1[px + 2]), "+v"(a1[px + 3]) : : "memory");
+        }
+#pragma unroll
+      for (int px = 0; px < R; ++px)
+        if (x0 + px < p.W) {
+          float v0, v1;
+          store2_stored<T>(out + (int64_t)(x0 + px) * p.Cout + n, a0[px] + w[CIN * 9 - 1].x * row[px + 2], a1[px] + w[CIN * 9 - 1].y * row[px + 2], v0, v1);
+          s0 += v0; q0 += v0 * v0; s1 += v1; q1 += v1 * v1;
+        }
+    }
+    *reinterpret_cast<float4*>(red + ((int64_t)wave * p.Cout + n) * 2) = make_float4(s0, q0, s1, q1);
+  }
+  if (p.sums == nullptr) return;
+  __syncthreads();
+  float* so = p.sums + (int64_t)(b * p.H + y) * p.Cout * 2;
+  for (int i = tid; i < p.Cout * 2; i += nthr) {
+    float a = 0.f;
+    for (int wv = 0; wv < nw; ++wv) a += red[(int64_t)wv * p.Cout * 2 + i];
+    so[i] = a;
+  }
+}
+
 constexpr int CONV_IN_PT = 8;
 template <typename T, int CIN>
-__global__ __launch_bounds__(128) void conv_in_kernel(ConvInParams p) {
+__global__ __launch_bounds__(128) void conv_in_ref_kernel(ConvInParams p) {
   constexpr int PT = CONV_IN_PT, PW = PT + 2;
   __shared__ float patch[CIN][3][PW];
   const int tid = threadIdx.x;
@@ -483,8 +575,11 @@
   return ns < 1 ? 1 : ns;
 }
 
+static std::atomic<long> g_gn_stats_launches{0};
+long gn_stats_launch_count() { return g_gn_stats_launches.load(); }
 int launch_gn_stats(const GnStatsParams& p, int dtype, hipStream_t s) {
   const int C = p.C0 + p.C1;
+  g_gn_stats_launches.fetch_add(1);
   if (p.groups != 32 || C % 128 != 0 || p.C0 % 4 != 0) return k22_set_error(K22_EINVAL, "gn_stats: need 32 groups, C % 128 == 0");
   if (C / 4 > 768) return k22_set_error(K22_EINVAL, "gn_stats: C too large (max 3072)");
   if (C / 4 < 256 && (256 / (C / 4)) * C > 2048) return k22_set_error(K22_EINVAL, "gn_stats: internal LDS bound");
@@ -527,22 +622,44 @@
   K22_CHECK_LAUNCH();
   return K22_OK;
 }
+template <typename T>
+static int launch_conv_in_t(const ConvInParams& p, dim3 grid, int threads, size_t lds, hipStream_t s) {
+  if (p.Cin == 4) hipLaunchKernelGGL((conv_in_kernel<T, 4>), grid, dim3(threads), lds, s, p);
+  else if (p.Cin == 9) hipLaunchKernelGGL((conv_in_kernel<T, 9>), grid, dim3(threads), lds, s, p);
+  else if (p.Cin == 8) hipLaunchKernelGGL((conv_in_kernel<T, 8>), grid, dim3(threads), lds, s, p);
+  else return k22_set_error(K22_EINVAL, "conv_in: in_channels must be 4, 8 or 9");
+  K22_CHECK_LAUNCH();
+  return K22_OK;
+}
 int launch_conv_in(const ConvInParams& p, int dtype, hipStream_t s) {
+  if (p.B < 1 || p.H < 1 || p.W < 1 || p.Cout < 2 || p.Cout % 2) return k22_set_error(K22_EINVAL, "conv_in: B, H, W >= 1 and an even Cout");
+  if (p.period < 1 || p.period > p.B) return k22_set_error(K22_EINVAL, "conv_in: period must be in [1, B]");
+  if (p.H > 65535 || p.B > 65535) return k22_set_error(K22_EINVAL, "conv_in: tensor too large");
+  const int nrun = (p.W + CONV_IN_R - 1) / CONV_IN_R;
+  const int nw = nrun < CONV_IN_MAX_WAVES ? nrun : CONV_IN_MAX_WAVES;
+  const size_t lds = ((size_t)p.Cin * 3 * (nrun * CONV_IN_R + 2) + (size_t)nw * p.Cout * 2) * sizeof(float);
+  if (lds > 64 * 1024) return k22_set_error(K22_EINVAL, "conv_in: row too wide / too many channels for the LDS (64 KB)");
+  const dim3 grid(p.H, p.B);
+  if (dtype == K22_BF16) return launch_conv_in_t<bf16_t>(p, grid, 64 * nw, lds, s);
+  if (dtype == K22_F16) return launch_conv_in_t<f16_t>(p, grid, 64 * nw, lds, s);
+  return launch_conv_in_t<float>(p, grid, 64 * nw, lds, s);
+}
+int launch_conv_in_reference(const ConvInParams& p, int dtype, hipStream_t s) {
   dim3 grid((p.W + CONV_IN_PT - 1) / CONV_IN_PT, p.H, p.B);
   if (p.Cin == 4) {
-    if (dtype == K22_BF16) hipLaunchKernelGGL((conv_in_kernel<bf16_t, 4>), grid, dim3(128), 0, s, p);
-    else if (dtype == K22_F16) hipLaunchKernelGGL((conv_in_kernel<f16_t, 4>), grid, dim3(128), 0, s, p);
-    else hipLaunchKernelGGL((conv_in_kernel<float, 4>), grid, dim3(128), 0, s, p);
+    if (dtype == K22_BF16) hipLaunchKernelGGL((conv_in_ref_kernel<bf16_t, 4>), grid, dim3(128), 0, s, p);
+    else if (dtype == K22_F16) hipLaunchKernelGGL((conv_in_ref_kernel<f16_t, 4>), grid, dim3(128), 0, s, p);
+    else hipLaunchKernelGGL((conv_in_ref_kernel<float, 4>), grid, dim3(128), 0, s, p);
   } else if (p.Cin == 9) {
-    if (dtype == K22_BF16) hipLaunchKernelGGL((conv_in_kernel<bf16_t, 9>), grid, dim3(128), 0, s, p);
-    else if (dtype == K22_F16) hipLaunchKernelGGL((conv_in_kernel<f16_t, 9>), grid, dim3(128), 0, s, p);
-    else hipLaunchKernelGGL((conv_in_kernel<float, 9>), grid, dim3(128), 0, s, p);
+    if (dtype == K22_BF16) hipLaunchKernelGGL((conv_in_ref_kernel<bf16_t, 9>), grid, dim3(128), 0, s, p);
+    else if (dtype == K22_F16) hipLaunchKernelGGL((conv_in_ref_kernel<f16_t, 9>), grid, dim3(128), 0, s, p);
+    else hipLaunchKernelGGL((conv_in_ref_kernel<float, 9>), grid, dim3(128), 0, s, p);
   } else if (p.Cin == 8) {
-    if (dtype == K22_BF16) hipLaunchKernelGGL((conv_in_kernel<bf16_t, 8>), grid, dim3(128), 0, s, p);
-    else if (dtype == K22_F16) hipLaunchKernelGGL((conv_in_kernel<f16_t, 8>), grid, dim3(128), 0, s, p);
-    else hipLaunchKernelGGL((conv_in_kernel<float, 8>), grid, dim3(128), 0, s, p);
+    if (dtype == K22_BF16) hipLaunchKernelGGL((conv_in_ref_kernel<bf16_t, 8>), grid, dim3(128), 0, s, p);
+    else if (dtype == K22_F16) hipLaunchKernelGGL((conv_in_ref_kernel<f16_t, 8>), grid, dim3(128), 0, s, p);
+    else hipLaunchKernelGGL((conv_in_ref_kernel<float, 8>), grid, dim3(128), 0, s, p);
   } else {
-    return k22_set_error(K22_EINVAL, "conv_in: in_channels must be 4, 8 or 9");
+    return k22_set_error(K22_EINVAL, "conv_in_reference: in_channels must be 4, 8 or 9");
   }
   K22_CHECK_LAUNCH();
   return K22_OK;
diff --git a/kandinsky-2_amd/csrc/engine.hip b/kandinsky-2_amd/csrc/engine.hip
--- a/kandinsky-2_amd/csrc/engine.hip
+++ b/kandinsky-2_amd/csrc/engine.hip
@@ -49,9 +49,11 @@
   Slot* s0 = nullptr; int C0 = 0;
   Slot* s1 = nullptr; int C1 = 0;
   int H = 0, W = 0;
-  const Tuned* p0 = nullptr; Slot* st0 = nullptr;
-  const Tuned* p1 = nullptr; Slot* st1 = nullptr;
+  const Tuned* p0 = nullptr; Slot* st0 = nullptr; int rpi0 = 0;
+  const Tuned* p1 = nullptr; Slot* st1 = nullptr; int rpi1 = 0;
   int C() const { return C0 + C1; }
+  int rows0() const { return p0 ? p0->rpi : rpi0; }
+  int rows1() const { return p1 ? p1->rpi : rpi1; }
 };
 
 }
@@ -101,6 +103,8 @@
   int hoist_time = 1;
   const float* film_cur = nullptr;
   const float* film_base() const { return film_cur ? film_cur : ptr<float>(s_film); }
+  const float* stem_x = nullptr;
+  int stem_period = 0;
   struct TimeW { const float* freqs; const float* w0; const float* b0; const float* w2; const float* b2; const void* we; const float* be; int mc, ted, dt; } tw = {};
   int time_rows(const float* t, float* temb, float* e1, float* emb, float* film, int rows, hipStream_t st) {
     int rc = launch_timestep_embedding(t, tw.freqs, temb, rows, tw.mc / 2, st);
@@ -173,9 +177,7 @@
     return K22_OK;
   }
   int loop_model(const LoopRows& lr, const float* cur, const float* timesteps, int call, hipStream_t s) {
-    const size_t half = (size_t)(B / 2) * 4 * H * W * sizeof(float);
-    if (int rc = copy_d2d(ptr(s_xin), cur, half, s)) return rc;
-    if (int rc = copy_d2d(ptr(s_xin) + half, cur, half, s)) return rc;
+    stem_x = cur; stem_period = B / 2;
     if (lr.hoist) {
       film_cur = lr.film + (int64_t)call * B * film_total;
     } else {
@@ -185,7 +187,7 @@
   }
   template <typename F> int loop_run(const std::vector<unsigned long long>& key, const float* timesteps, const float* inpaint_image,
                                      const float* inpaint_mask, int use_graph, hipStream_t st, F body) {
-    auto run_loop = [&](hipStream_t s) -> int { const int rc = body(s); film_cur = nullptr; return rc; };
+    auto run_loop = [&](hipStream_t s) -> int { const int rc = body(s); film_cur = nullptr; stem_x = nullptr; return rc; };
     if (!use_graph) {
       const int rc = run_loop(st);
       if (rc == K22_OK) loop_count_launch();
@@ -241,8 +243,8 @@
       const void* x1 = a.s1 ? ptr(a.s1) : nullptr;
       GnCoeffParams cp = {};
       if (fused) {
-        cp.src[0].st = ptr<float>(a.st0); cp.src[0].rpi = a.p0->rpi; cp.src[0].C = a.C0;
-        if (a.s1) { cp.src[1].st = ptr<float>(a.st1); cp.src[1].rpi = a.p1->rpi; cp.src[1].C = a.C1; }
+        cp.src[0].st = ptr<float>(a.st0); cp.src[0].rpi = a.rows0(); cp.src[0].C = a.C0;
+        if (a.s1) { cp.src[1].st = ptr<float>(a.st1); cp.src[1].rpi = a.rows1(); cp.src[1].C = a.C1; }
         if (cp.src[0].rpi <= 0 || (a.s1 && cp.src[1].rpi <= 0)) return k22_set_error(K22_EINVAL, "unet: producer delivered no GroupNorm partial sums");
       } else {
         GnStatsParams sp;
@@ -561,6 +563,8 @@
     int ch = mc * cfg.channel_mult[0];
     {
       Slot* d = new_slot((size_t)B * H * W * ch * esz);
+      const int stem_rpi = conv_in_rows_per_image(H, W);
+      Slot* dst_st = new_slot((size_t)B * stem_rpi * ch * 2 * sizeof(float));
       ConvInParams cp = {};
       cp.w = Wf("input_blocks.0.0.weight"); cp.bias = Wf("input_blocks.0.0.bias");
       cp.B = B; cp.H = H; cp.W = W; cp.Cin = cfg.in_channels; cp.Cout = ch;
@@ -568,12 +572,15 @@
       const int premul = (hinted || cfg.head_type == 1) ? 1 : 0;
       ops.push_back([=](hipStream_t st) {
         ConvInParams q = cp;
-        q.x = ptr<float>(s_xin); q.img = inpaint ? ptr<float>(s_img) : (hinted ? ptr<float>(s_hint) : nullptr);
+        q.x = stem_x ? stem_x : ptr<float>(s_xin); q.period = stem_x ? stem_period : cp.B;
+        q.sums = ptr<float>(dst_st);
+        q.img = inpaint ? ptr<float>(s_img) : (hinted ? ptr<float>(s_hint) : nullptr);
         q.mask = inpaint ? ptr<float>(s_mask) : nullptr; q.img_premul = premul;
         q.out = ptr(d);
         return launch_conv_in(q, dt, st);
       });
       Act a; a.s0 = d; a.C0 = ch; a.H = H; a.W = W;
+      a.st0 = dst_st; a.rpi0 = stem_rpi;
       hs.push_back(a);
     }
     Act h = hs.back();
@@ -612,7 +619,7 @@
       for (int i = 0; i <= cfg.num_res_blocks; ++i) {
         const Act skip = hs.back(); hs.pop_back();
         Act cat; cat.s0 = h.s0; cat.C0 = h.C0; cat.s1 = skip.s0; cat.C1 = skip.C0; cat.H = h.H; cat.W = h.W;
-        cat.p0 = h.p0; cat.st0 = h.st0; cat.p1 = skip.p0; cat.st1 = skip.st0;
+        cat.p0 = h.p0; cat.st0 = h.st0; cat.rpi0 = h.rpi0; cat.p1 = skip.p0; cat.st1 = skip.st0; cat.rpi1 = skip.rpi0;
         if (skip.H != h.H || skip.W != h.W) return k22_set_error(K22_EINVAL, "unet: skip shape mismatch");
         const int co = mc * cfg.channel_mult[l];
         const std::string pfx = "output_blocks." + std::to_string(blk);
diff --git a/kandinsky-2_amd/csrc/igemm.hip b/kandinsky-2_amd/csrc/igemm.hip
--- a/kandinsky-2_amd/csrc/igemm.hip
+++ b/kandinsky-2_amd/csrc/igemm.hip
@@ -443,6 +443,12 @@
       if (L.splitk < 1) L.splitk = 1;
       L.block = 256; L.grid = (unsigned)nb; L.lds = stream_lds_bytes(p, mb);
     }
+  }
+  if (!L.algo && p.algo == IG_ALGO_SMALLN) {
+    if (!conv3_smalln_supported(p, dtype)) return k22_set_error(K22_EINVAL, "igemm: the small-N convolution kernel (algo 21) does not run this problem");
+    if (p.stats != nullptr) return k22_set_error(K22_EINVAL, "igemm: the small-N convolution kernel writes no GroupNorm partial sums");
+    L.family = IG_FAM_SMALLN; L.algo = IG_ALGO_SMALLN; L.bm = 128; L.bn = 8; L.splitk = 1; L.block = 512;
+    L.grid = conv3_smalln_grid(p); L.lds = conv3_smalln_lds_bytes(p);
   }
   const int conv_algo = (p.algo && p.algo != IG_ALGO_STREAM) ? p.algo : (o.conv_algo == IG_ALGO_STREAM ? 0 : o.conv_algo);
   if (!L.algo && p.taps == 9 && conv_algo != IG_ALGO_GENERIC && p.N >= 128 && !p.a_raw) {
@@ -564,7 +570,7 @@
   L.finish = !finishes ? IG_FINISH_NONE : (reduce_rows_ok(p, p.stats != nullptr) ? IG_FINISH_ROWS : IG_FINISH_FLAT);
   if (p.taps == 1 && (generic || p.H <= 0 || qkv)) L.stats_rows_per_image = 0;
   else if (finishes) L.stats_rows_per_image = reduce_rows_ok(p, true) ? p.H * p.W / 16 : 0;
-  else if (generic) L.stats_rows_per_image = 0;
+  else if (generic || L.family == IG_FAM_SMALLN) L.stats_rows_per_image = 0;
   else L.stats_rows_per_image = p.taps == 1 ? gemm8_tiles_per_image(p, L.bm) : conv3_halo_tiles_per_image(p, L.bm);
   *out = L;
   return K22_OK;
@@ -654,6 +660,7 @@
     case IG_FAM_GEMM8: case IG_FAM_GEMM8_SPEC: rc = launch_gemm8(q, dtype, L, stream); break;
     case IG_FAM_SPEC: rc = launch_conv3_halo_spec(q, dtype, L, stream); break;
     case IG_FAM_GENERIC: rc = launch_generic(q, dtype, L, stream); break;
+    case IG_FAM_SMALLN: rc = launch_conv3_smalln(q, dtype, L, stream); break;
     default: rc = launch_conv3_halo(q, dtype, L, stream); break;
   }
   if (rc || L.finish == IG_FINISH_NONE) return rc;
diff --git a/kandinsky-2_amd/csrc/kernels.h b/kandinsky-2_amd/csrc/kernels.h
--- a/kandinsky-2_amd/csrc/kernels.h
+++ b/kandinsky-2_amd/csrc/kernels.h
@@ -77,11 +77,13 @@
   IG_ALGO_SPEC_PIPE = 12,
   IG_ALGO_DBG_SPEC_NO_DMA = 13,
   IG_ALGO_DBG_SPEC_NO_WAIT = 14,
-  IG_ALGO_STREAM = 20
+  IG_ALGO_STREAM = 20,
+  IG_ALGO_SMALLN = 21
 };
 struct IgemmAlgoName { int algo; const char* name; };
 constexpr IgemmAlgoName IGEMM_ALGO_NAMES[] = {{IG_ALGO_GENERIC, "gen"},   {IG_ALGO_HALO, "halo"},   {IG_ALGO_HALO3, "hal3"}, {IG_ALGO_HALO_PIPE, "hal6"},
-                                              {IG_ALGO_HALO_ASM, "hal7"}, {IG_ALGO_GEMM8, "gem8"}, {IG_ALGO_SPEC, "spec"},  {IG_ALGO_SPEC_PIPE, "spcp"}};
+                                              {IG_ALGO_HALO_ASM, "hal7"}, {IG_ALGO_GEMM8, "gem8"}, {IG_ALGO_SPEC, "spec"},  {IG_ALGO_SPEC_PIPE, "spcp"},
+                                              {IG_ALGO_SMALLN, "smln"}};
 inline const char* igemm_algo_name(int algo) {
   for (const IgemmAlgoName& a : IGEMM_ALGO_NAMES) if (a.algo == algo) return a.name;
   return "auto";
@@ -102,7 +104,7 @@
   return p;
 }
 
-enum IgemmFamily { IG_FAM_GENERIC, IG_FAM_HALO, IG_FAM_HALO3, IG_FAM_SPEC, IG_FAM_GEMM8, IG_FAM_GEMM8_SPEC, IG_FAM_STREAM };
+enum IgemmFamily { IG_FAM_GENERIC, IG_FAM_HALO, IG_FAM_HALO3, IG_FAM_SPEC, IG_FAM_GEMM8, IG_FAM_GEMM8_SPEC, IG_FAM_STREAM, IG_FAM_SMALLN };
 enum IgemmFinish { IG_FINISH_NONE, IG_FINISH_FLAT, IG_FINISH_ROWS };
 struct IgemmLaunch {
   int family;
@@ -143,6 +145,10 @@
 int launch_conv3_halo(const IgemmParams& p, int dtype, const IgemmLaunch& L, hipStream_t stream);
 int launch_conv3_halo_spec(const IgemmParams& p, int dtype, const IgemmLaunch& L, hipStream_t stream);
 int launch_conv3_halo_trace(const IgemmParams& p, int dtype, hipStream_t stream);
+bool conv3_smalln_supported(const IgemmParams& p, int dtype);
+size_t conv3_smalln_lds_bytes(const IgemmParams& p);
+unsigned conv3_smalln_grid(const IgemmParams& p);
+int launch_conv3_smalln(const IgemmParams& p, int dtype, const IgemmLaunch& L, hipStream_t stream);
 bool gemm8_supported(const IgemmParams& p, int dtype, int bm);
 bool gemm8_spec_supported(int dtype);
 int gemm8_tiles_per_image(const IgemmParams& p, int bm);
diff --git a/kandinsky-2_amd/csrc/tuning.h b/kandinsky-2_amd/csrc/tuning.h
--- a/kandinsky-2_amd/csrc/tuning.h
+++ b/kandinsky-2_amd/csrc/tuning.h
@@ -139,6 +139,10 @@
       }
     }
   }
+  if (conv3_smalln_supported(p, dtype)) {
+    Cfg c; c.algo = IG_ALGO_SMALLN; c.bm = 128; c.bn = 0; c.splitk = 1; c.stages = 0;
+    all.push_back(c);
+  }
   const int tiles[3][2] = {{128, 128}, {128, 64}, {64, 64}};
   const bool skinny = p.taps == 1;
   for (auto& tl : tiles) {
```

Result: no change. 149.5 steps/s (median of 6 runs) (+0.8%).
